# ZulutionAI/MoviiGen1.1

Measured on AMD Instinct MI355X. Metric: denoise-steps/sec, higher is better.
Workload: dtype bf16; 1 GPU; 14B T2V 1920x832x81f bf16 (the metric's configuration; BASELINE configs[2] shape); layers=40, parallelism=single, solver=unipc, weights=random N(0,0.02) bf16, seed 0

## Files before the change

### experiments/mfma_shape_probe.hip

```cpp
#include <hip/hip_runtime.h>
#include <stdio.h>
#include <stdlib.h>
#include <string.h>
#include <vector>

typedef __attribute__((ext_vector_type(8))) __bf16 bf16x8_t;
typedef __attribute__((ext_vector_type(16))) float f32x16_t;
typedef __attribute__((ext_vector_type(4))) float f32x4_t;
typedef __attribute__((ext_vector_type(4))) unsigned int u32x4_t;
#define CK(x) do { hipError_t e_ = (x); if (e_ != hipSuccess) { printf("HIP error %s at %d\n", hipGetErrorString(e_), __LINE__); exit(1); } } while (0)
#define SB() __builtin_amdgcn_sched_barrier(0)

template <int SHAPE, int FILL, int WAVES, int RDS = 1>
__global__ __launch_bounds__(WAVES * 64, 1) void mix(const u32x4_t* __restrict__ in, float* __restrict__ out, int iters,
                                                     unsigned long long* __restrict__ cyc) {
    __shared__ __attribute__((aligned(16))) char smem[96 * 1024];
    const int tid = threadIdx.x, lane = tid & 63;
    for (int i = tid; i < 4096; i += WAVES * 64) ((u32x4_t*)smem)[i] = in[i];
    __syncthreads();
    bf16x8_t a[4], b[4];
#pragma unroll
    for (int i = 0; i < 4; ++i) {
        a[i] = __builtin_bit_cast(bf16x8_t, in[(tid * 4 + i) & 4095]);
        b[i] = __builtin_bit_cast(bf16x8_t, in[(tid * 4 + i + 1777) & 4095]);
    }
    f32x16_t A32[4];
    f32x4_t A16[16];
#pragma unroll
    for (int i = 0; i < 4; ++i)
#pragma unroll
        for (int e = 0; e < 16; ++e) A32[i][e] = 0.f;
#pragma unroll
    for (int i = 0; i < 16; ++i) A16[i] = (f32x4_t){0.f, 0.f, 0.f, 0.f};
    float x[4] = {0.001f * lane, -0.002f * lane, 0.5f, -0.25f}, y[4] = {0, 0, 0, 0}, s0 = 0.f, s1 = 0.f;
    unsigned pk = 0;
    const char* lp = smem + lane * 16;
    auto fill_a = [&](int k) __attribute__((always_inline)) {
        asm volatile("v_exp_f32 %0, %1" : "=v"(y[k & 3]) : "v"(x[k & 3]));
        asm volatile("v_add_f32 %0, %0, %1" : "+v"(s0) : "v"(y[(k + 2) & 3]));
    };
    auto fill_b = [&](int k) __attribute__((always_inline)) {
        asm volatile("v_exp_f32 %0, %1" : "=v"(y[(k + 1) & 3]) : "v"(x[(k + 1) & 3]));
        asm volatile("v_add_f32 %0, %0, %1" : "+v"(s1) : "v"(y[(k + 3) & 3]));
        asm volatile("v_cvt_pk_bf16_f32 %0, %1, %2" : "=v"(pk) : "v"(y[k & 3]), "v"(y[(k + 2) & 3]));
    };
    const unsigned long long t0 = __builtin_amdgcn_s_memtime();
    for (int it = 0; it < iters; ++it) {
#pragma unroll
        for (int j = 0; j < 8; ++j) {
            if (SHAPE == 0) {
                A32[(2 * j) & 3] = __builtin_amdgcn_mfma_f32_32x32x16_bf16(a[j & 3], b[j & 3], A32[(2 * j) & 3], 0, 0, 0);
                SB();
#pragma unroll
                for (int f = 0; f < FILL; ++f) fill_a(j + f);
                SB();
                A32[(2 * j + 1) & 3] = __builtin_amdgcn_mfma_f32_32x32x16_bf16(a[j & 3], b[(j + 1) & 3], A32[(2 * j + 1) & 3], 0, 0, 0);
                SB();
#pragma unroll
                for (int f = 0; f < FILL; ++f) fill_b(j + f);
            } else {
                A16[(4 * j) & 15] = __builtin_amdgcn_mfma_f32_16x16x32_bf16(a[j & 3], b[j & 3], A16[(4 * j) & 15], 0, 0, 0);
                SB();
#pragma unroll
                for (int f = 0; f < FILL; ++f) asm volatile("v_exp_f32 %0, %1" : "=v"(y[(j + f) & 3]) : "v"(x[(j + f) & 3]));
                SB();
                A16[(4 * j + 1) & 15] = __builtin_amdgcn_mfma_f32_16x16x32_bf16(a[j & 3], b[(j + 1) & 3], A16[(4 * j + 1) & 15], 0, 0, 0);
                SB();
#pragma unroll
                for (int f = 0; f < FILL; ++f) {
                    asm volatile("v_add_f32 %0, %0, %1" : "+v"(s0) : "v"(y[(j + f + 2) & 3]));
                    asm volatile("v_add_f32 %0, %0, %1" : "+v"(s1) : "v"(y[(j + f + 3) & 3]));
                }
                SB();
                A16[(4 * j + 2) & 15] = __builtin_amdgcn_mfma_f32_16x16x32_bf16(a[j & 3], b[(j + 2) & 3], A16[(4 * j + 2) & 15], 0, 0, 0);
                SB();
#pragma unroll
                for (int f = 0; f < FILL; ++f) asm volatile("v_exp_f32 %0, %1" : "=v"(y[(j + f + 1) & 3]) : "v"(x[(j + f + 1) & 3]));
                SB();
                A16[(4 * j + 3) & 15] = __builtin_amdgcn_mfma_f32_16x16x32_bf16(a[j & 3], b[(j + 3) & 3], A16[(4 * j + 3) & 15], 0, 0, 0);
                SB();
#pragma unroll
                for (int f = 0; f < FILL; ++f)
                    asm volatile("v_cvt_pk_bf16_f32 %0, %1, %2" : "=v"(pk) : "v"(y[(j + f) & 3]), "v"(y[(j + f + 2) & 3]));
            }
            if (FILL >= 0) a[(j + 2) & 3] = *(const bf16x8_t*)(lp + ((j * 1024 + it * 8192) & 0xfc00));
            if (RDS >= 2) b[(j + 2) & 3] = *(const bf16x8_t*)(lp + ((j * 1024 + it * 8192 + 32768) & 0xfc00));
            SB();
        }
    }
    const unsigned long long t1 = __builtin_amdgcn_s_memtime();
    float r = s0 + s1 + __uint_as_float(pk);
#pragma unroll
    for (int i = 0; i < 4; ++i)
#pragma unroll
        for (int e = 0; e < 16; ++e) r += A32[i][e];
#pragma unroll
    for (int i = 0; i < 16; ++i) r += A16[i][0] + A16[i][1] + A16[i][2] + A16[i][3];
    out[blockIdx.x * WAVES * 64 + tid] = r;
    if (tid == 0) cyc[blockIdx.x] = t1 - t0;
}

template <int SHAPE, int FILL, int WAVES, int RDS = 1>
static void run(const u32x4_t* in, float* out, unsigned long long* cyc, int rounds) {
    const int iters = 20000, grid = 1024;
    for (int r = 0; r < rounds; ++r) {
        hipEvent_t e0, e1;
        CK(hipEventCreate(&e0)); CK(hipEventCreate(&e1));
        hipLaunchKernelGGL((mix<SHAPE, FILL, WAVES, RDS>), dim3(grid), dim3(WAVES * 64), 0, 0, in, out, 2000, cyc);
        CK(hipDeviceSynchronize());
        CK(hipEventRecord(e0));
        hipLaunchKernelGGL((mix<SHAPE, FILL, WAVES, RDS>), dim3(grid), dim3(WAVES * 64), 0, 0, in, out, iters, cyc);
        CK(hipEventRecord(e1));
        CK(hipEventSynchronize(e1));
        float ms;
        CK(hipEventElapsedTime(&ms, e0, e1));
        std::vector<unsigned long long> h(grid);
        CK(hipMemcpy(h.data(), cyc, grid * 8, hipMemcpyDeviceToHost));
        double cs = 0;
        for (auto v : h) cs += (double)v;
        cs /= grid;
        const double flops = (double)grid * WAVES * iters * 8 * 65536.0;
        printf("%s  waves/CU %d  fill x%d (VALU per 32x32x16-equivalent: %.1f) + %.1f ds_read: %8.1f TF/s  %6.1f cyc per 32768 FLOP  (clock ~%.2f GHz)\n",
               SHAPE ? "16x16x32" : "32x32x16", WAVES, FILL, FILL * 2.5, 0.5 * RDS, flops / (ms * 1e-3) / 1e12, cs / (iters * 16.0),
               cs * (grid / 256.0) / (ms * 1e-3) / 1e9 / 1.0);
        fflush(stdout);
    }
}

int main() {
    u32x4_t* in; float* out; unsigned long long* cyc;
    CK(hipMalloc(&in, 65536)); CK(hipMalloc(&out, 1024 * 512 * 4)); CK(hipMalloc(&cyc, 1024 * 8));
    std::vector<unsigned short> h(32768);
    srand(1);
    for (auto& v : h) {
        float f = ((rand() % 2001) - 1000) / 1000.0f;
        unsigned u; memcpy(&u, &f, 4);
        v = (unsigned short)(u >> 16);
    }
    CK(hipMemcpy(in, h.data(), 65536, hipMemcpyHostToDevice));
    for (int round = 0; round < 2; ++round) {
        run<0, 0, 4>(in, out, cyc, 1);
        run<1, 0, 4>(in, out, cyc, 1);
        run<0, 1, 4>(in, out, cyc, 1);
        run<1, 1, 4>(in, out, cyc, 1);
        run<0, 2, 4>(in, out, cyc, 1);
        run<1, 2, 4>(in, out, cyc, 1);
        run<0, 1, 8>(in, out, cyc, 1);
        run<1, 1, 8>(in, out, cyc, 1);
        run<1, 1, 8, 2>(in, out, cyc, 1);
        run<1, 1, 4, 2>(in, out, cyc, 1);
    }
    return 0;
}
```

### include/moviigen_hip.h

```cpp
#ifndef MOVIIGEN_HIP_H
#define MOVIIGEN_HIP_H

#include <stdint.h>

#ifdef __cplusplus
extern "C" {
#endif

#define MG_OK 0
#define MG_ERR_ARG (-1)
#define MG_ERR_SHAPE (-2)
#define MG_ERR_LAUNCH (-3)
#define MG_ERR_UNAVAILABLE (-4)
#define MG_ERR_COMM (-5)

const char* mg_version(void);
int mg_abi_version(void);


int mg_ln_modulate(const float* x, int64_t ldx, int64_t rows, int dim, const float* scale,
                   const float* shift, int add_one, float eps, int round_norm_bf16, void* out,
                   int out_f32, int64_t ldo, void* stream);

int64_t mg_step_resid_partials_bytes(void);
int mg_step_resid_capture_f32(float* r, const float* x, const float* xin, int64_t n, double* stats, double* partials,
                              void* stream);
int mg_resid_ln_modulate_f32(const float* x, int64_t ldx, const float* r, int64_t ldr, int64_t rows, int dim,
                             const float* scale, const float* shift, float eps, float* out, int64_t ldo, void* stream);

int mg_rmsnorm_rope_bf16(const uint16_t* x, int64_t ldx, uint16_t* out, int64_t ldo,
                         int64_t rows, int dim, const float* weight, float eps, int head_dim,
                         const float* rope_cs, int F, int H, int W, int64_t pos0, float out_scale, void* stream);

int mg_pack_kv_bf16(const uint16_t* k, int64_t ldk, const uint16_t* v, int64_t ldv, int64_t L,
                    int heads, int head_dim, uint16_t* kp, uint16_t* vp, void* stream);


enum {
    MG_EPI_BIAS_BF16 = 0,
    MG_EPI_BIAS_GELU_BF16 = 1,
    MG_EPI_GATE_RESID_F32 = 2,
    MG_EPI_BIAS_F32 = 3
};

int mg_gemm_bf16(const uint16_t* A, int64_t lda, const uint16_t* W, int64_t ldw,
                 const float* bias, int64_t M, int N, int K, int epilogue, void* out,
                 int64_t ldo, const float* gate, void* stream);

int mg_quant_mxfp8_rows(const uint16_t* x, int64_t ldx, int64_t rows, int K, uint8_t* q, int64_t ldq,
                        uint8_t* scales, int64_t lds, void* stream);

int mg_gemm_mxfp8(const uint8_t* Aq, int64_t lda, const uint8_t* As, int64_t ldas, const uint8_t* Wq, int64_t ldw,
                  const uint8_t* Ws, int64_t ldws, const float* bias, int64_t M, int N, int K, int epilogue,
                  void* out, int64_t ldo, const float* gate, void* stream);

int mg_ln_modulate_mxfp8(const float* x, int64_t ldx, int64_t rows, int dim, const float* scale, const float* shift,
                         int add_one, float eps, int round_norm_bf16, uint16_t* out, int64_t ldo, uint8_t* q,
                         int64_t ldq, uint8_t* scales, int64_t lds, void* stream);

int mg_gemm_mxfp8_gelu_q(const uint8_t* Aq, int64_t lda, const uint8_t* As, int64_t ldas, const uint8_t* Wq, int64_t ldw,
                         const uint8_t* Ws, int64_t ldws, const float* bias, int64_t M, int N, int K, uint8_t* oq,
                         int64_t ldoq, uint8_t* oscales, int64_t ldos, void* stream);

int64_t mg_attn_workspace_bytes(void);
int mg_attn_fwd_bf16_hd128(const uint16_t* q, int64_t ldq, const uint16_t* kp, const uint16_t* vp,
                           uint16_t* o, int64_t ldo, int64_t Lq, int64_t Lk, int heads, float scale,
                           void* workspace, void* stream);

int mg_attn_fwd_bf16_hd128_lse(const uint16_t* q, int64_t ldq, const uint16_t* kp, const uint16_t* vp,
                               uint16_t* o, int64_t ldo, float* lse, int64_t Lq, int64_t Lk, int heads,
                               float scale, void* workspace, void* stream);

int mg_attn_fwd_bf16_hd128_prescaled(const uint16_t* q, int64_t ldq, const uint16_t* kp, const uint16_t* vp,
                                     uint16_t* o, int64_t ldo, float* lse, int64_t Lq, int64_t Lk, int heads,
                                     int reserve_cus, void* workspace, void* stream);

int mg_gate_residual_f32(float* x, int64_t ldx, const uint16_t* y, int64_t ldy, const float* gate, int64_t rows,
                         int dim, void* stream);


int mg_sp_pack_qkv_bf16(const uint16_t* q, int64_t ldq, const uint16_t* k, int64_t ldk, const uint16_t* v,
                        int64_t ldv, int64_t Lloc, int P, int cols_per_dest, int col0, int w, uint16_t* send,
                        void* stream);

int mg_sp_unpack_o_bf16(const uint16_t* recv, int64_t Lloc, int P, int cols_per_src, int col0, int w, uint16_t* o,
                        int64_t ldo, void* stream);

int mg_sp_copy_blocks_bf16(const uint16_t* src, int64_t s_blk, int64_t s_row, uint16_t* dst, int64_t d_blk,
                           int64_t d_row, int blocks, int64_t rows, int width, void* stream);


int mg_comm_unique_id(void* id128);
int mg_comm_create(const void* id128, int nranks, int rank, void** comm);
int mg_comm_destroy(void* comm);

int mg_sp_all_to_all(void* comm, const void* send, void* recv, int64_t bytes_per_peer, void* stream);

int mg_sp_all_to_all_4d_bf16(void* comm, const uint16_t* x, int64_t ldx, int64_t rows, int heads, int head_dim,
                             int seq_to_head, uint16_t* out, int64_t ldo, uint16_t* workspace, void* stream);

int mg_sp_all_gather(void* comm, const void* send, void* recv, int64_t bytes, void* stream);
int mg_shard_all_gather(void* comm, const void* shard, void* full, int64_t shard_bytes, void* stream);

int mg_attn_merge_f32(float* acc, int64_t lda, float* lse_acc, const uint16_t* part, int64_t ldp,
                      const float* lse_part, uint16_t* out, int64_t ldo, int64_t Lq, int heads, int first,
                      void* stream);

int mg_attn_fwd_bf16_generic(const uint16_t* q, int64_t ldq, const uint16_t* k, int64_t ldk,
                             const uint16_t* v, int64_t ldv, uint16_t* o, int64_t ldo, int64_t Lq,
                             int64_t Lk, int heads, int head_dim, float scale, void* stream);


int mg_sinusoid_embed(const void* t, int t_dtype, int n, int dim, float* out, void* stream);

int mg_gemv_f32(const float* W, const float* bias, const float* x, float* y, int N, int K,
                int silu_in, void* stream);

int mg_add_rows_f32(const float* a, const float* b, float* out, int rows, int dim, int period,
                    void* stream);

int mg_head_gemm_f32(const float* x, int64_t ldx, const float* W, const float* bias, float* out,
                     int64_t M, int N, int K, void* stream);

int mg_patchify_bf16(const float* lat, int C, int F, int H, int W, int ph, int pw,
                     uint16_t* out, int64_t ldo, void* stream);

int mg_unpatchify_f32(const float* tok, int64_t ldt, int C, int F, int Hg, int Wg, int ph, int pw,
                      float* lat, void* stream);

int mg_lincomb4_f32(float* out, int64_t n, const float* x0, float c0, const float* x1, float c1,
                    const float* x2, float c2, const float* x3, float c3, void* stream);

int mg_cfg_combine_f32(float* out, const float* uncond, const float* cond, float guide_scale,
                       int64_t n, void* stream);


int mg_embed_rows_bf16(const uint16_t* table, int64_t vocab, int dim, const int64_t* ids, int n,
                       uint16_t* out, void* stream);

int mg_ew_bf16(const uint16_t* a, const uint16_t* b, uint16_t* out, int64_t n, int mode, void* stream);

int mg_t5_attn_bf16(const uint16_t* q, const uint16_t* k, const uint16_t* v, int64_t ld,
                    const uint16_t* rel_emb, const int* rel_bucket, uint16_t* o, int64_t ldo,
                    int64_t Lq, int64_t Lk, int heads, int head_dim, void* stream);


int mg_vae_conv_f32(const float* x, const float* cache, int tc, int T, int H, int W, int Cin,
                    const float* w, const float* bias, int Cout, int kt, int kh, int kw, int up2,
                    const float* residual, float* out, int mode, void* stream);

int mg_vae_upconv_fold_weights_f32(const float* w, int Cout, int Cin, float* wp, void* stream);
int mg_vae_upconv_phases_f32(const float* x, int T, int H, int W, int Cin, const float* wp, const float* bias, int Cout,
                             float* out, int mode, void* stream);

int mg_vae_conv_cols_f32(const float* x, const float* cache, int tc, int T, int H, int W, int Cin,
                         const float* w, const float* bias, int Cout, int kt, int kh, int kw,
                         const float* residual, float* out, int col0, int cols, int mode, void* stream);
int mg_vae_upconv_phases_cols_f32(const float* x, int T, int H, int W, int Cin, const float* wp, const float* bias, int Cout,
                                  float* out, int col0, int cols, int mode, void* stream);

#define MG_VAE_EXACT 0
#define MG_VAE_BF16X3 1
#define MG_VAE_TILE_128 (1 << 8)
#define MG_VAE_TILE_256 (2 << 8)

int mg_vae_rmsnorm_silu_f32(const float* x, const float* gamma, float* out, int64_t rows, int C,
                            int do_silu, void* stream);

int64_t mg_vae_attn_workspace_floats(int64_t L, int C);
int mg_vae_attn_f32(const float* qkv, float* out, int frames, int64_t L, int C, float* workspace,
                    void* stream);
int mg_vae_attn_rows_f32(const float* q, int64_t ldq, const float* k, const float* v, int64_t ldkv, float* out, int frames,
                         int64_t Lq, int64_t Lk, int C, float* workspace, void* stream);

int mg_vae_latent_in_f32(const float* z, const float* mean, const float* inv_std, int C, int T,
                         int H, int W, float* out, void* stream);
int mg_vae_video_out_f32(const float* x, int C, int T, int H, int W, float* out, int t_off,
                         int T_total, void* stream);

int mg_video_to_u8(const float* video, int T, int H, int W, float lo, float hi, uint8_t* frames,
                   void* stream);

int mg_image_to_u8(const float* image, int H, int W, float lo, float hi, uint8_t* pixels, void* stream);

int mg_video_from_u8(const uint8_t* frames, int T, int H0, int W0, int H, int W, float* video, void* stream);

int mg_vae_time_interleave_f32(const float* x, int T, int64_t HW, int C, float* out, void* stream);


int mg_vae_conv_strided_f32(const float* x, const float* cache, int tc, int T, int H, int W, int Cin, const float* w, const float* bias,
                            int Cout, int kt, int kh, int kw, int st, int sh, int sw, int pt0, int ph0, int ph1, int pw0, int pw1,
                            float* out, int mode, void* stream);

int mg_vae_conv_in3_f32(const float* xs, const float* cache, int tc, int T, int H, int W, const float* w, const float* bias, int Cout,
                        float* out, int mode, void* stream);

int mg_vae_video_in_f32(const float* video, int T, int H, int W, int t0, int n, float* out, void* stream);
int mg_vae_latent_out_f32(const float* x, int ldx, const float* mean, const float* inv_std, int C, int T, int H, int W, float* out,
                          void* stream);


int mg_lora_merge(void* w, int w_f32, int64_t ldw, int N, int K, const float* up, int64_t ldu, const float* down, int64_t ldd, int R,
                  void* stream);

#ifdef MG_AB_BUILD
int mg_gemm_set_variant(int variant);

int mg_attn_set_variant(int variant);

void mg_attn_w64_profile(unsigned long long* dev_buf);
void mg_attn_w64_debug(int flags);
void mg_attn_w64_flag_counter(unsigned* dev_counter);
void mg_gemm_debug_profile(unsigned long long* dev_buf);
void mg_gemm5_debug_profile(unsigned long long* dev_buf);
#endif

#ifdef __cplusplus
}
#endif
#endif
```

### moviigen1.1_amd/csrc/attn_hd128_m16.hip

```cpp
#include <type_traits>
#include "common.h"
#include "../../include/moviigen_hip.h"

#define M16_THREADS 256
#define M16_QB 256
#define M16_TILE 16384
#define M16_K(slot) ((slot) * M16_TILE)
#define M16_V(slot) (3 * M16_TILE + (slot) * M16_TILE)

MG_DEV bf16x8_t m16_bf(u32x4_t v) { return __builtin_bit_cast(bf16x8_t, v); }
struct M16State {
    f32x4_t ot[8][4];
    f32x4_t st[2][2][4];
    bf16x8_t pf[2][4];
    f32x4_t mq[4];
    float m_run[4], l_run[4];
    float psa[4], psb[4];
    int bad;
};

template <int OFF>
MG_DEV void m16_rd(bf16x8_t& dst, unsigned addr) {
    asm volatile("ds_read_b128 %0, %1 offset:%2" : "=v"(dst) : "v"(addr), "i"(OFF));
}
template <int N>
MG_DEV void m16_wait() {
    asm volatile("s_waitcnt lgkmcnt(%0)" ::"i"(N) : "memory");
}
MG_DEV void m16_mfma_s0(f32x4_t& acc, const bf16x8_t& a, const bf16x8_t& b, const f32x4_t& c) {
    asm volatile("v_mfma_f32_16x16x32_bf16 %0, %1, %2, %3" : "=&v"(acc) : "v"(a), "a"(b), "v"(c));
}
MG_DEV void m16_mfma_s(f32x4_t& acc, const bf16x8_t& a, const bf16x8_t& b) {
    asm volatile("v_mfma_f32_16x16x32_bf16 %0, %1, %2, %0" : "+v"(acc) : "v"(a), "a"(b));
}
MG_DEV void m16_mfma_s_after_valu(f32x4_t& acc, const bf16x8_t& a, const bf16x8_t& b) {
    asm volatile("s_nop 7\n\ts_nop 7\n\tv_mfma_f32_16x16x32_bf16 %0, %1, %2, %0" : "+v"(acc) : "v"(a), "a"(b));
}
constexpr int m16_koff(int i) { return (i >> 2) * 256 + (i & 3) * 4096; }
constexpr int m16_voff(int i) { return i * 256; }

template <int KB>
MG_DEV void m16_softmax_exact(M16State& s, float c) {
#pragma unroll
    for (int n = 0; n < 4; ++n) {
        float tmax = s.st[KB][0][n][0];
#pragma unroll
        for (int r = 1; r < 4; ++r) tmax = fmaxf(tmax, s.st[KB][0][n][r]);
#pragma unroll
        for (int r = 0; r < 4; ++r) tmax = fmaxf(tmax, s.st[KB][1][n][r]);
        tmax = fmaxf(tmax, __shfl_xor(tmax, 16, 64));
        tmax = fmaxf(tmax, __shfl_xor(tmax, 32, 64));
        const float m_new = fmaxf(s.m_run[n], tmax);
        float psum = 0.f;
        float p[8];
#pragma unroll
        for (int r = 0; r < 8; ++r) {
            p[r] = __builtin_amdgcn_exp2f((s.st[KB][r >> 2][n][r & 3] - m_new) * c);
            psum += p[r];
        }
        u32x4_t w;
#pragma unroll
        for (int e = 0; e < 4; ++e) w[e] = pack_bf2(p[2 * e], p[2 * e + 1]);
        s.pf[KB][n] = m16_bf(w);
        const float alpha = __builtin_amdgcn_exp2f((s.m_run[n] - m_new) * c);
        s.l_run[n] = s.l_run[n] * alpha + psum;
#pragma unroll
        for (int d = 0; d < 8; ++d)
#pragma unroll
            for (int e = 0; e < 4; ++e) s.ot[d][n][e] *= alpha;
        s.m_run[n] = m_new;
    }
}

template <int KB>
MG_DEV void m16_softmax_zero(M16State& s, float c) {
#pragma unroll
    for (int n = 0; n < 4; ++n) {
        float psum = 0.f;
        float p[8];
#pragma unroll
        for (int r = 0; r < 8; ++r) {
            p[r] = __builtin_amdgcn_exp2f(s.st[KB][r >> 2][n][r & 3] * c);
            psum += p[r];
        }
        u32x4_t w;
#pragma unroll
        for (int e = 0; e < 4; ++e) w[e] = pack_bf2(p[2 * e], p[2 * e + 1]);
        s.pf[KB][n] = m16_bf(w);
        s.l_run[n] += psum;
    }
}

template <int KB>
MG_DEV void m16_mask_init(M16State& s, int lim, int G, const f32x4_t (&base)[4]) {
#pragma unroll
    for (int blk = 0; blk < 2; ++blk)
#pragma unroll
        for (int n = 0; n < 4; ++n)
#pragma unroll
            for (int r = 0; r < 4; ++r) {
                const int key = KB * 32 + G * 8 + blk * 4 + r;
                s.st[KB][blk][n][r] = key >= lim ? -1e30f : base[n][0];
            }
}

template <int KB, int SMODE, bool PV, bool SM, bool SCALED, int ORD, int LKO = 0, int LVO = 0, int NKO = 0, int NVO = 0, typename Dma>
MG_DEV void m16_step(M16State& s, const bf16x8_t (&qf)[4][4], bf16x8_t (&kf)[4], bf16x8_t (&vf)[4], unsigned lds_k,
                     unsigned lds_v, unsigned nk, unsigned nv, float c, Dma dma) {
    constexpr int SB = 1 - KB;
    u32x4_t w[4];
    float pa[2] = {0.f, 0.f}, pb[2] = {0.f, 0.f};
    auto exp_a = [&](int i, int half) __attribute__((always_inline)) {
        if (SM) {
            const int pp = 2 * i + half, n = pp >> 2, wd = pp & 3;
            const float x = s.st[SB][wd >> 1][n][(wd & 1) * 2];
            pa[half] = __builtin_amdgcn_exp2f(SCALED ? x * c : x);
            asm volatile("" : "+v"(pa[half]));
        }
    };
    auto exp_b = [&](int i, int half) __attribute__((always_inline)) {
        if (SM) {
            const int pp = 2 * i + half, n = pp >> 2, wd = pp & 3;
            const float x = s.st[SB][wd >> 1][n][(wd & 1) * 2 + 1];
            pb[half] = __builtin_amdgcn_exp2f(SCALED ? x * c : x);
            asm volatile("" : "+v"(pb[half]));
        }
    };
    auto add_a = [&](int i, int half) __attribute__((always_inline)) {
        if (SM) {
            const int n = (2 * i + half) >> 2;
            s.psa[n] += pa[half];
            asm volatile("" : "+v"(s.psa[n]));
        }
    };
    auto add_b = [&](int i, int half) __attribute__((always_inline)) {
        if (SM) {
            const int n = (2 * i + half) >> 2;
            s.psb[n] += pb[half];
            asm volatile("" : "+v"(s.psb[n]));
        }
    };
    auto cvt = [&](int i, int half) __attribute__((always_inline)) {
        if (SM) {
            const int pp = 2 * i + half, n = pp >> 2, wd = pp & 3;
            unsigned pk = pack_bf2(pa[half], pb[half]);
            asm volatile("" : "+v"(pk));
            w[n][wd] = pk;
        }
    };
    auto S = [&](int i, int n) __attribute__((always_inline)) {
        const int blk = i >> 2, c = i & 3, r = i & 3;
        if (SMODE == 1 && c == 0) m16_mfma_s0(s.st[KB][blk][n], kf[r], qf[n][c], s.mq[n]);
        else if (SMODE == 2 && c == 0) m16_mfma_s_after_valu(s.st[KB][blk][n], kf[r], qf[n][c]);
        else if (SMODE != 0) m16_mfma_s(s.st[KB][blk][n], kf[r], qf[n][c]);
    };
    auto P = [&](int i, int n) __attribute__((always_inline)) {
        if (PV) s.ot[i][n] = __builtin_amdgcn_mfma_f32_16x16x32_bf16(vf[i & 3], s.pf[KB][n], s.ot[i][n], 0, 0, 0);
    };
    auto rdK = [&](int i) __attribute__((always_inline)) {
        const int r2 = (i + 2) & 3;
        if (SMODE == 0) asm volatile("" ::"v"(kf[r2]));
        if (i < 6) {
            switch (i) {
                case 0: m16_rd<m16_koff(2) + LKO>(kf[r2], lds_k); break;
                case 1: m16_rd<m16_koff(3) + LKO>(kf[r2], lds_k); break;
                case 2: m16_rd<m16_koff(4) + LKO>(kf[r2], lds_k); break;
                case 3: m16_rd<m16_koff(5) + LKO>(kf[r2], lds_k); break;
                case 4: m16_rd<m16_koff(6) + LKO>(kf[r2], lds_k); break;
                default: m16_rd<m16_koff(7) + LKO>(kf[r2], lds_k); break;
            }
        } else if (i == 6) m16_rd<m16_koff(0) + NKO>(kf[r2], nk);
        else m16_rd<m16_koff(1) + NKO>(kf[r2], nk);
    };
    auto rdV = [&](int i) __attribute__((always_inline)) {
        const int r2 = (i + 2) & 3;
        if (i < 6) {
            switch (i) {
                case 0: m16_rd<m16_voff(2) + LVO>(vf[r2], lds_v); break;
                case 1: m16_rd<m16_voff(3) + LVO>(vf[r2], lds_v); break;
                case 2: m16_rd<m16_voff(4) + LVO>(vf[r2], lds_v); break;
                case 3: m16_rd<m16_voff(5) + LVO>(vf[r2], lds_v); break;
                case 4: m16_rd<m16_voff(6) + LVO>(vf[r2], lds_v); break;
                default: m16_rd<m16_voff(7) + LVO>(vf[r2], lds_v); break;
            }
        } else if (i == 6) m16_rd<m16_voff(0) + NVO>(vf[r2], nv);
        else m16_rd<m16_voff(1) + NVO>(vf[r2], nv);
    };
#define M16_SB() __builtin_amdgcn_sched_barrier(0)
#pragma unroll
    for (int i = 0; i < 8; ++i) {
        m16_wait<2>();
        M16_SB();
        if constexpr (ORD == 0) {
            S(i, 0); M16_SB();
            exp_a(i, 0); exp_b(i, 0); M16_SB();
            P(i, 0); M16_SB();
            add_a(i, 0); add_b(i, 0); cvt(i, 0); M16_SB();
            S(i, 1); M16_SB();
            rdK(i); M16_SB();
            P(i, 1); M16_SB();
            rdV(i); M16_SB();
            S(i, 2); M16_SB();
            exp_a(i, 1); exp_b(i, 1); M16_SB();
            P(i, 2); M16_SB();
            add_a(i, 1); add_b(i, 1); cvt(i, 1); M16_SB();
            S(i, 3); M16_SB();
            dma(i); M16_SB();
            P(i, 3); M16_SB();
        } else if constexpr (ORD == 1) {
            S(i, 0); M16_SB();
            exp_a(i, 0); M16_SB();
            P(i, 0); M16_SB();
            exp_b(i, 0); M16_SB();
            S(i, 1); M16_SB();
            add_a(i, 0); add_b(i, 0); cvt(i, 0); M16_SB();
            P(i, 1); M16_SB();
            rdK(i); M16_SB(); rdV(i); M16_SB();
            S(i, 2); M16_SB();
            exp_a(i, 1); M16_SB();
            P(i, 2); M16_SB();
            exp_b(i, 1); M16_SB();
            S(i, 3); M16_SB();
            add_a(i, 1); add_b(i, 1); cvt(i, 1); M16_SB();
            P(i, 3); M16_SB();
            dma(i); M16_SB();
        } else if constexpr (ORD == 2) {
            S(i, 0); M16_SB();
            exp_a(i, 0); M16_SB(); rdK(i); M16_SB();
            P(i, 0); M16_SB();
            exp_b(i, 0); M16_SB(); rdV(i); M16_SB();
            S(i, 1); M16_SB();
            add_a(i, 0); add_b(i, 0); cvt(i, 0); M16_SB();
            P(i, 1); M16_SB();
            S(i, 2); M16_SB();
            exp_a(i, 1); M16_SB();
            P(i, 2); M16_SB();
            exp_b(i, 1); M16_SB();
            S(i, 3); M16_SB();
            add_a(i, 1); add_b(i, 1); cvt(i, 1); M16_SB();
            P(i, 3); M16_SB();
            dma(i); M16_SB();
        } else if constexpr (ORD == 4) {
            S(i, 0); M16_SB();
            exp_a(i, 0); M16_SB();
            P(i, 0); M16_SB();
            exp_b(i, 0); M16_SB();
            S(i, 1); M16_SB();
            add_a(i, 0); add_b(i, 0); M16_SB();
            P(i, 1); M16_SB();
            cvt(i, 0); M16_SB(); rdK(i); M16_SB(); rdV(i); M16_SB();
            S(i, 2); M16_SB();
            exp_a(i, 1); M16_SB();
            P(i, 2); M16_SB();
            exp_b(i, 1); M16_SB();
            S(i, 3); M16_SB();
            add_a(i, 1); add_b(i, 1); M16_SB();
            P(i, 3); M16_SB();
            cvt(i, 1); M16_SB(); dma(i); M16_SB();
        } else if constexpr (ORD == 5) {
            S(i, 0); M16_SB();
            exp_a(i, 0); M16_SB();
            P(i, 0); M16_SB();
            exp_b(i, 0); M16_SB();
            S(i, 1); M16_SB();
            add_a(i, 0); add_b(i, 0); cvt(i, 0); M16_SB();
            P(i, 1); M16_SB();
            rdK(i); M16_SB();
            S(i, 2); M16_SB();
            exp_a(i, 1); M16_SB();
            P(i, 2); M16_SB();
            exp_b(i, 1); M16_SB();
            S(i, 3); M16_SB();
            add_a(i, 1); add_b(i, 1); cvt(i, 1); M16_SB();
            P(i, 3); M16_SB();
            rdV(i); M16_SB(); dma(i); M16_SB();
        } else if constexpr (ORD == 8) {
            S(i, 0); M16_SB();
            exp_a(i, 0); M16_SB();
            S(i, 1); M16_SB();
            exp_b(i, 0); M16_SB();
            P(i, 0); M16_SB();
            add_a(i, 0); add_b(i, 0); cvt(i, 0); M16_SB();
            P(i, 1); M16_SB();
            rdK(i); M16_SB(); rdV(i); M16_SB();
            S(i, 2); M16_SB();
            exp_a(i, 1); M16_SB();
            S(i, 3); M16_SB();
            exp_b(i, 1); M16_SB();
            P(i, 2); M16_SB();
            add_a(i, 1); add_b(i, 1); cvt(i, 1); M16_SB();
            P(i, 3); M16_SB();
            dma(i); M16_SB();
        } else if constexpr (ORD == 9) {
            S(i, 0); M16_SB();
            exp_a(i, 0); M16_SB();
            S(i, 1); M16_SB();
            exp_b(i, 0); M16_SB();
            S(i, 2); M16_SB();
            add_a(i, 0); add_b(i, 0); cvt(i, 0); M16_SB();
            S(i, 3); M16_SB();
            rdK(i); M16_SB(); rdV(i); M16_SB();
            P(i, 0); M16_SB();
            exp_a(i, 1); M16_SB();
            P(i, 1); M16_SB();
            exp_b(i, 1); M16_SB();
            P(i, 2); M16_SB();
            add_a(i, 1); add_b(i, 1); cvt(i, 1); M16_SB();
            P(i, 3); M16_SB();
            dma(i); M16_SB();
        } else {
            S(i, 0); M16_SB();
            exp_a(i, 0); M16_SB();
            P(i, 0); M16_SB();
            exp_b(i, 0); M16_SB();
            S(i, 1); M16_SB();
            exp_a(i, 1); M16_SB();
            P(i, 1); M16_SB();
            exp_b(i, 1); M16_SB();
            S(i, 2); M16_SB();
            add_a(i, 0); add_b(i, 0); cvt(i, 0); M16_SB();
            P(i, 2); M16_SB();
            add_a(i, 1); add_b(i, 1); cvt(i, 1); M16_SB();
            S(i, 3); M16_SB();
            rdK(i); M16_SB(); rdV(i); M16_SB();
            P(i, 3); M16_SB();
            dma(i); M16_SB();
        }
    }
#undef M16_SB
    if (SM) {
#pragma unroll
        for (int n = 0; n < 4; ++n) {
            s.pf[SB][n] = m16_bf(w[n]);
        }
    }
}

MG_DEV int m16_lane() {
    int l;
    asm volatile("v_mbcnt_lo_u32_b32 %0, -1, 0\n\tv_mbcnt_hi_u32_b32 %0, -1, %0" : "=v"(l));
    return l;
}

struct M16NoDma {
    __device__ __forceinline__ void operator()(int) const {}
};

template <bool PROF, bool SCALED, int ORD>
__global__ __launch_bounds__(M16_THREADS, 1) void attn_hd128_m16_kernel(
    const uint16_t* __restrict__ q, int64_t ldq, const uint16_t* __restrict__ kp, const uint16_t* __restrict__ vp,
    uint16_t* __restrict__ o, int64_t ldo, int64_t Lq, int64_t Lk, int heads, float c_log2, int nqb, int dbg,
    unsigned long long* __restrict__ prof, float* __restrict__ lse, unsigned* __restrict__ flagcnt, unsigned* __restrict__ tickets) {
    __shared__ __attribute__((aligned(16))) char smem[6 * M16_TILE];
    __shared__ int s_next_item;
    const int bid = blockIdx.x;
    const unsigned long long r_start = PROF ? __builtin_amdgcn_s_memrealtime() : 0;
    const int tid = threadIdx.x;
    const int wave = __builtin_amdgcn_readfirstlane(tid >> 6);
    const int total_items = nqb * heads;
    const int nwg = gridDim.x;
    const bool ticketed = tickets != nullptr && nwg != total_items;
    int item, item_end, item_step;
    if (nwg == total_items || ticketed) {
        item = bid, item_end = ticketed ? total_items : bid + 1, item_step = 1;
    } else {
        const int xcd = bid & 7, slot = bid >> 3;
        item = (int)((int64_t)xcd * total_items / 8) + slot;
        item_end = (int)((int64_t)(xcd + 1) * total_items / 8);
        item_step = nwg >> 3;
    }
    unsigned next_ticket = 0;
    unsigned long long ph[8] = {0, 0, 0, 0, 0, 0, 0, 0}, ph_t = 0;
    unsigned long long pf_fence = 0, pf_a = 0, pf_b = 0, pf_n = 0;
    while (item < item_end) {
    if (ticketed && tid == 0) next_ticket = atomicAdd(tickets, 1u);
    const int head = item / nqb;
    const int qb0 = item - head * nqb;
    const int lane = m16_lane();
    int qi = lane & 15, G = lane >> 4;
    __syncthreads();
    if (PROF) ph_t = __builtin_amdgcn_s_memtime();

    bf16x8_t qf[4][4];
    const int64_t qrow_base = (int64_t)qb0 * M16_QB + wave * 64 + qi;
#pragma unroll
    for (int n = 0; n < 4; ++n) {
        const int64_t qr = qrow_base + n * 16;
        const int64_t qrow = qr < Lq ? qr : Lq - 1;
        const uint16_t* qp = q + qrow * ldq + head * 128 + G * 8;
#pragma unroll
        for (int c = 0; c < 4; ++c) qf[n][c] = m16_bf(*(const u32x4_t*)(qp + c * 32));
    }
    const int T = (int)((Lk + 63) / 64);
    const int last_lim = (int)(Lk - (int64_t)(T - 1) * 64);
    const int nfull = last_lim == 64 ? T : T - 1;
    const unsigned lds0 = (unsigned)(uintptr_t)(mg_lptr_t)smem;
    const uint64_t kb64 = (uint64_t)(uintptr_t)(kp + ((int64_t)head * T) * 8192), vb64 = (uint64_t)(uintptr_t)(vp + ((int64_t)head * T) * 8192);
    const u32x4_t rs_k = {(unsigned)__builtin_amdgcn_readfirstlane((int)(unsigned)kb64), (unsigned)__builtin_amdgcn_readfirstlane((int)((unsigned)(kb64 >> 32) & 0xffffu)),
                          (unsigned)T * M16_TILE, 0x00020000u};
    const u32x4_t rs_v = {(unsigned)__builtin_amdgcn_readfirstlane((int)(unsigned)vb64), (unsigned)__builtin_amdgcn_readfirstlane((int)((unsigned)(vb64 >> 32) & 0xffffu)),
                          (unsigned)T * M16_TILE, 0x00020000u};
    const int dvo = wave * 4096 + lane * 16;
    const unsigned lds_w = (unsigned)__builtin_amdgcn_readfirstlane((int)(lds0 + wave * 4096));
    auto dma_tile4 = [&](const u32x4_t& rs, int t, unsigned lbase) __attribute__((always_inline)) {
        const int soff = __builtin_amdgcn_readfirstlane((t < T ? t : T - 1) * M16_TILE);
        asm volatile("s_mov_b32 m0, %2\n\ts_nop 4\n\t"
                     "buffer_load_dwordx4 %0, %1, %3 offen lds\n\t"
                     "buffer_load_dwordx4 %0, %1, %3 offen offset:1024 lds\n\t"
                     "buffer_load_dwordx4 %0, %1, %3 offen offset:2048 lds\n\t"
                     "buffer_load_dwordx4 %0, %1, %3 offen offset:3072 lds"
                     :: "v"(dvo), "s"(rs), "s"(lbase), "s"(soff) : "memory");
    };
    auto dma_k4 = [&](int t, int slot) __attribute__((always_inline)) { dma_tile4(rs_k, t, lds_w + M16_K(slot)); };
    auto dma_v4 = [&](int t, int slot) __attribute__((always_inline)) { dma_tile4(rs_v, t, lds_w + M16_V(slot)); };
    unsigned kbase = lds0 + G * 1024 + qi * 16;
    unsigned vbase = lds0 + 3 * M16_TILE + G * 2048 + qi * 16;
    auto k_addr = [&](int slot, int kb) __attribute__((always_inline)) { return kbase + slot * M16_TILE + kb * 512; };
    auto v_addr = [&](int slot, int kb) __attribute__((always_inline)) { return vbase + slot * M16_TILE + kb * 8192; };

    M16State s;
    bf16x8_t kf[4], vf[4];
    auto reset = [&]() __attribute__((always_inline)) {
#pragma unroll
        for (int d = 0; d < 8; ++d)
#pragma unroll
            for (int n = 0; n < 4; ++n) s.ot[d][n] = (f32x4_t){0.f, 0.f, 0.f, 0.f};
#pragma unroll
        for (int n = 0; n < 4; ++n) s.m_run[n] = -1e30f, s.l_run[n] = 0.f, s.psa[n] = 0.f, s.psb[n] = 0.f;
        s.bad = 0;
    };
    reset();
    auto q_pin = [&]() __attribute__((always_inline)) {
#pragma unroll
        for (int n = 0; n < 4; ++n)
#pragma unroll
            for (int c = 0; c < 4; ++c) asm volatile("" : "+a"(qf[n][c]));
    };
    auto fence = [&]() __attribute__((always_inline)) {
        asm volatile("s_waitcnt vmcnt(0)" ::: "memory");
        __syncthreads();
    };
    auto fence_hot = [&]() __attribute__((always_inline)) {
        asm volatile("s_waitcnt vmcnt(0)\n\ts_barrier" ::: "memory");
    };
    auto prefetch = [&](unsigned ak, unsigned av) __attribute__((always_inline)) {
        m16_rd<m16_koff(0)>(kf[0], ak);
        m16_rd<m16_voff(0)>(vf[0], av);
        m16_rd<m16_koff(1)>(kf[1], ak);
        m16_rd<m16_voff(1)>(vf[1], av);
    };
    const f32x4_t zero4[4] = {{0.f, 0.f, 0.f, 0.f}, {0.f, 0.f, 0.f, 0.f}, {0.f, 0.f, 0.f, 0.f}, {0.f, 0.f, 0.f, 0.f}};
    auto bare_S = [&](auto kbc, int slot, int lim) __attribute__((always_inline)) {
        constexpr int KB = decltype(kbc)::value;
        if (lim < 64) m16_mask_init<KB>(s, lim, G, zero4);
        else {
#pragma unroll
            for (int blk = 0; blk < 2; ++blk)
#pragma unroll
                for (int n = 0; n < 4; ++n) s.st[KB][blk][n] = (f32x4_t){0.f, 0.f, 0.f, 0.f};
        }
        const char* base = smem + M16_K(slot) + G * 1024 + qi * 16 + KB * 512;
#pragma unroll
        for (int i = 0; i < 8; ++i) {
            const bf16x8_t f = *(const bf16x8_t*)(base + m16_koff(i));
#pragma unroll
            for (int n = 0; n < 4; ++n)
                s.st[KB][i >> 2][n] = __builtin_amdgcn_mfma_f32_16x16x32_bf16(f, qf[n][i & 3], s.st[KB][i >> 2][n], 0, 0, 0);
        }
    };
    auto bare_PV = [&](auto kbc, int slot) __attribute__((always_inline)) {
        constexpr int KB = decltype(kbc)::value;
        const char* base = smem + M16_V(slot) + G * 2048 + qi * 16 + KB * 8192;
#pragma unroll
        for (int i = 0; i < 8; ++i) {
            const bf16x8_t f = *(const bf16x8_t*)(base + m16_voff(i));
#pragma unroll
            for (int n = 0; n < 4; ++n)
                s.ot[i][n] = __builtin_amdgcn_mfma_f32_16x16x32_bf16(f, s.pf[KB][n], s.ot[i][n], 0, 0, 0);
        }
    };
    using KB0 = std::integral_constant<int, 0>;
    using KB1 = std::integral_constant<int, 1>;

    bool exact_pass = nfull < 3;
    if (!exact_pass) {
    for (int attempt = 0;; ++attempt) {
        auto tile_max = [&](float (&mx)[4]) __attribute__((always_inline)) {
#pragma unroll
            for (int n = 0; n < 4; ++n) {
                float a = fmaxf(fmaxf(s.st[0][0][n][0], s.st[0][0][n][1]), fmaxf(s.st[0][0][n][2], s.st[0][0][n][3]));
                float b = fmaxf(fmaxf(s.st[0][1][n][0], s.st[0][1][n][1]), fmaxf(s.st[0][1][n][2], s.st[0][1][n][3]));
                float c2 = fmaxf(fmaxf(s.st[1][0][n][0], s.st[1][0][n][1]), fmaxf(s.st[1][0][n][2], s.st[1][0][n][3]));
                float d2 = fmaxf(fmaxf(s.st[1][1][n][0], s.st[1][1][n][1]), fmaxf(s.st[1][1][n][2], s.st[1][1][n][3]));
                mx[n] = fmaxf(mx[n], fmaxf(fmaxf(a, b), fmaxf(c2, d2)));
            }
        };
        auto set_reference = [&](const float (&mx)[4], float above) __attribute__((always_inline)) {
#pragma unroll
            for (int n = 0; n < 4; ++n) {
                float m = fmaxf(mx[n], __shfl_xor(mx[n], 16, 64));
                m = fmaxf(m, __shfl_xor(m, 32, 64)) + above;
                s.mq[n] = (f32x4_t){-m, -m, -m, -m};
            }
        };
        if (attempt) {
            float mx[4] = {-1e30f, -1e30f, -1e30f, -1e30f};
#pragma unroll
            for (int a = 0; a < 4; ++a) dma_k4(a, a);
            for (int t = 0; t < T; ++t) {
                asm volatile("s_waitcnt vmcnt(12)" ::: "memory");
                __syncthreads();
                dma_k4(t + 4, (t + 4) % 6);
                const int lim = t == T - 1 ? last_lim : 64;
                bare_S(KB0{}, t % 6, lim);
                bare_S(KB1{}, t % 6, lim);
                tile_max(mx);
            }
            asm volatile("s_waitcnt vmcnt(0)" ::: "memory");
            set_reference(mx, 0.f);
            __syncthreads();
            reset();
        }
        dma_k4(0, 0), dma_v4(0, 0), dma_k4(1, 1);
        fence();
        q_pin();
        if (PROF) { const unsigned long long tt = __builtin_amdgcn_s_memtime(); ph[0] += tt - ph_t; ph_t = tt; }
        dma_k4(2, 2), dma_v4(1, 1);
        bare_S(KB0{}, 0, 64);
        bare_S(KB1{}, 0, 64);
        if (attempt == 0) {
            float mx[4] = {-1e30f, -1e30f, -1e30f, -1e30f};
            tile_max(mx);
            set_reference(mx, c_log2 > 1e-20f ? 64.f / c_log2 : 0.f);
        }
#pragma unroll
        for (int kb = 0; kb < 2; ++kb)
#pragma unroll
            for (int blk = 0; blk < 2; ++blk)
#pragma unroll
                for (int n = 0; n < 4; ++n) s.st[kb][blk][n] += s.mq[n];
        m16_softmax_zero<0>(s, c_log2);
#pragma unroll
        for (int n = 0; n < 4; ++n) asm volatile("" : "+v"(s.l_run[n]));
        prefetch(k_addr(1, 0), v_addr(0, 0));
        m16_step<0, 1, true, true, SCALED, ORD>(s, qf, kf, vf, k_addr(1, 0), v_addr(0, 0), k_addr(1, 1), v_addr(0, 1), c_log2, M16NoDma());
        int t = 1;
        unsigned ka0 = k_addr(0, 0), ka1 = k_addr(1, 0), ka2 = k_addr(2, 0);
        unsigned va0 = v_addr(0, 0), va1 = v_addr(1, 0), va2 = v_addr(2, 0);
        unsigned lk0 = (unsigned)__builtin_amdgcn_readfirstlane((int)(lds0 + M16_K(0) + wave * 4096));
        unsigned lk1 = lk0 + M16_TILE, lk2 = lk0 + 2 * M16_TILE;
        int offk = (t + 2) * M16_TILE, offv = (t + 1) * M16_TILE;
        unsigned keep_m0, rot_tmp;
#define M16_BDMA0(VOFF, RS, SOFF, LBASE, IMM)                                                                                              \
    asm volatile("s_add_u32 m0, %2, %3\n\ts_nop 0\n\tbuffer_load_dwordx4 %0, %1, %4 offen lds"                                             \
                 :: "v"(VOFF), "s"(RS), "s"(LBASE), "n"(IMM), "s"(SOFF) : "memory", "scc")
#define M16_BDMAN(VOFF, RS, SOFF, IMM)                                                                                                     \
    asm volatile("buffer_load_dwordx4 %0, %1, %3 offen offset:%2 lds" :: "v"(VOFF), "s"(RS), "n"(IMM), "s"(SOFF) : "memory")
        asm volatile("s_mov_b32 %0, m0\n\ts_nop 4" : "=s"(keep_m0) :: "memory");
        if (PROF) { const unsigned long long tt = __builtin_amdgcn_s_memtime(); ph[1] += tt - ph_t; ph_t = tt; }
        __builtin_amdgcn_s_waitcnt(0x0F70);
        asm volatile("" : "+v"(ka0), "+v"(ka1), "+v"(ka2), "+v"(va0), "+v"(va1), "+v"(va2));
        if (PROF) { const unsigned long long tt = __builtin_amdgcn_s_memtime(); ph[2] += tt - ph_t; ph_t = tt; }
        for (; t + 1 < nfull; ++t) {
            const unsigned long long c0 = PROF ? __builtin_amdgcn_s_memtime() : 0;
            fence_hot();
            const unsigned long long c1 = PROF ? __builtin_amdgcn_s_memtime() : 0;
            m16_step<1, 1, true, true, SCALED, ORD, 512, 8192, 0, 0>(s, qf, kf, vf, ka1, va0, ka2, va1, c_log2,
                                       [&](int n) __attribute__((always_inline)) {
                                           switch (n) {
                                               case 0: M16_BDMA0(dvo, rs_k, offk, lk0, 0); break;
                                               case 1: M16_BDMAN(dvo, rs_k, offk, 1024); break;
                                               case 2: M16_BDMAN(dvo, rs_k, offk, 2048); break;
                                               case 3: M16_BDMAN(dvo, rs_k, offk, 3072); break;
                                               case 4: M16_BDMA0(dvo, rs_v, offv, lk2, 3 * M16_TILE); break;
                                               case 5: M16_BDMAN(dvo, rs_v, offv, 1024); break;
                                               case 6: M16_BDMAN(dvo, rs_v, offv, 2048); break;
                                               default: M16_BDMAN(dvo, rs_v, offv, 3072); break;
                                           }
                                       });
            const unsigned long long c2 = PROF ? __builtin_amdgcn_s_memtime() : 0;
            m16_step<0, 1, true, true, SCALED, ORD, 0, 0, 512, 8192>(s, qf, kf, vf, ka2, va1, ka2, va1, c_log2,
                                       [&](int n) __attribute__((always_inline)) {
                                           if (n == 0)
                                               asm volatile("s_add_u32 %0, %0, 0x4000\n\ts_add_u32 %1, %1, 0x4000" : "+s"(offk), "+s"(offv) : : "scc");
                                           else if (n == 1)
                                               asm volatile("s_mov_b32 %3, %0\n\ts_mov_b32 %0, %1\n\ts_mov_b32 %1, %2\n\ts_mov_b32 %2, %3"
                                                            : "+s"(lk0), "+s"(lk1), "+s"(lk2), "=&s"(rot_tmp));
                                           else if (n == 7) {
                                               asm volatile("v_swap_b32 %0, %1\n\tv_swap_b32 %1, %2" : "+v"(ka0), "+v"(ka1), "+v"(ka2));
                                               asm volatile("v_swap_b32 %0, %1\n\tv_swap_b32 %1, %2" : "+v"(va0), "+v"(va1), "+v"(va2));
                                           }
                                       });
            if (PROF) {
                const unsigned long long c3 = __builtin_amdgcn_s_memtime();
                pf_fence += c1 - c0, pf_a += c2 - c1, pf_b += c3 - c2, pf_n += 1;
            }
        }
#undef M16_BDMA0
#undef M16_BDMAN
        asm volatile("s_mov_b32 m0, %0" :: "s"(keep_m0) : "memory");
        if (PROF) { const unsigned long long tt = __builtin_amdgcn_s_memtime(); ph[3] += tt - ph_t; ph_t = tt; }
        static_assert(M16_TILE == 0x4000, "the literal above");
        const int s0 = (t - 1) % 3, s1 = t % 3, s2 = (t + 1) % 3;
        {
            const int l2 = m16_lane();
            qi = l2 & 15, G = l2 >> 4;
            kbase = lds0 + G * 1024 + qi * 16;
            vbase = lds0 + 3 * M16_TILE + G * 2048 + qi * 16;
        }
        fence();
        if (t + 1 < T) {
            dma_v4(t + 1, s2);
        }
        m16_step<1, 1, true, true, SCALED, ORD>(s, qf, kf, vf, k_addr(s1, 1), v_addr(s0, 1), k_addr(s2, 0), v_addr(s1, 0), c_log2, M16NoDma());
        if (t + 1 < T) {
            m16_mask_init<0>(s, last_lim, G, s.mq);
            m16_step<0, 2, true, true, SCALED, ORD>(s, qf, kf, vf, k_addr(s2, 0), v_addr(s1, 0), k_addr(s2, 1), v_addr(s1, 1), c_log2, M16NoDma());
            fence();
            m16_mask_init<1>(s, last_lim, G, s.mq);
            m16_step<1, 2, true, true, SCALED, ORD>(s, qf, kf, vf, k_addr(s2, 1), v_addr(s1, 1), k_addr(s2, 1), v_addr(s2, 0), c_log2, M16NoDma());
            m16_step<0, 0, true, true, SCALED, ORD>(s, qf, kf, vf, k_addr(s2, 1), v_addr(s2, 0), k_addr(s2, 1), v_addr(s2, 1), c_log2, M16NoDma());
            m16_step<1, 0, true, false, SCALED, ORD>(s, qf, kf, vf, k_addr(s2, 1), v_addr(s2, 1), k_addr(s2, 1), v_addr(s2, 1), c_log2, M16NoDma());
        } else {
            m16_step<0, 0, true, true, SCALED, ORD>(s, qf, kf, vf, k_addr(s1, 1), v_addr(s1, 0), k_addr(s1, 1), v_addr(s1, 1), c_log2, M16NoDma());
            m16_step<1, 0, true, false, SCALED, ORD>(s, qf, kf, vf, k_addr(s1, 1), v_addr(s1, 1), k_addr(s1, 1), v_addr(s1, 1), c_log2, M16NoDma());
        }
        m16_wait<0>();
        asm volatile("" ::"v"(kf[0]), "v"(kf[1]), "v"(kf[2]), "v"(kf[3]), "v"(vf[0]), "v"(vf[1]), "v"(vf[2]), "v"(vf[3]));
#pragma unroll
        for (int n = 0; n < 4; ++n) {
            s.l_run[n] += s.psa[n] + s.psb[n];
            s.psa[n] = s.psb[n] = 0.f;
            float lt = s.l_run[n] + __shfl_xor(s.l_run[n], 16, 64);
            lt += __shfl_xor(lt, 32, 64);
            s.bad |= !(lt >= 8.4703295e-22f && lt <= 1.2379400e27f);
            s.m_run[n] = -s.mq[n][0];
        }
        const bool flagged = __syncthreads_or(s.bad) != 0;
        if (PROF) { const unsigned long long tt = __builtin_amdgcn_s_memtime(); ph[4] += tt - ph_t; ph_t = tt; }
        if (!flagged || (dbg & 1)) break;
        if (flagcnt && tid == 0) atomicAdd(flagcnt + (attempt ? 1 : 0), 1u);
        if (attempt) {
            exact_pass = true;
            break;
        }
    }
    }
    if (exact_pass) {
        reset();
        for (int t = 0; t < T; ++t) {
            __syncthreads();
            dma_k4(t, 0), dma_v4(t, 0);
            fence();
            q_pin();
            const int lim = t == T - 1 ? last_lim : 64;
            bare_S(KB0{}, 0, lim);
            bare_S(KB1{}, 0, lim);
            m16_softmax_exact<0>(s, c_log2);
            bare_PV(KB0{}, 0);
            m16_softmax_exact<1>(s, c_log2);
            bare_PV(KB1{}, 0);
        }
    }

    {
        const int l3 = m16_lane();
        qi = l3 & 15, G = l3 >> 4;
    }
#pragma unroll
    for (int n = 0; n < 4; ++n) {
        float l_tot = s.l_run[n] + __shfl_xor(s.l_run[n], 16, 64);
        l_tot += __shfl_xor(l_tot, 32, 64);
        const float inv = 1.f / l_tot;
        const int64_t qr = (int64_t)qb0 * M16_QB + wave * 64 + n * 16 + qi;
        if (lse && G == 0 && qr < Lq) lse[(int64_t)head * Lq + qr] = (s.m_run[n] * c_log2 + __log2f(l_tot)) * 0.6931471805599453f;
        if (qr < Lq) {
            uint16_t* op = o + qr * ldo + head * 128 + G * 4;
#pragma unroll
            for (int d = 0; d < 8; ++d) {
                uint2 pk;
                pk.x = pack_bf2(s.ot[d][n][0] * inv, s.ot[d][n][1] * inv);
                pk.y = pack_bf2(s.ot[d][n][2] * inv, s.ot[d][n][3] * inv);
                *(uint2*)(op + d * 16) = pk;
            }
        }
    }
    if (PROF) { ph[7] += __builtin_amdgcn_s_memtime() - ph_t; asm volatile("s_waitcnt vmcnt(0)" ::: "memory"); const unsigned long long tt = __builtin_amdgcn_s_memtime(); ph[5] += tt - ph_t; ph[6] += 1; }
    if (ticketed) {
        if (tid == 0) s_next_item = nwg + (int)next_ticket;
        __syncthreads();
        item = __builtin_amdgcn_readfirstlane(s_next_item);
    } else
        item += item_step;
    }
    if (ticketed && tid == 0 && atomicAdd(tickets + 1, 1u) == (unsigned)nwg - 1) {
        __hip_atomic_store(tickets, 0u, __ATOMIC_RELAXED, __HIP_MEMORY_SCOPE_AGENT);
        __hip_atomic_store(tickets + 1, 0u, __ATOMIC_RELAXED, __HIP_MEMORY_SCOPE_AGENT);
    }
    if (PROF && prof && tid == 0) prof[16 + 2 * bid] = r_start, prof[16 + 2 * bid + 1] = __builtin_amdgcn_s_memrealtime();
    if (PROF && prof && (tid & 63) == 0) {
        atomicAdd(prof + wave * 4 + 0, pf_fence);
        atomicAdd(prof + wave * 4 + 1, pf_a);
        atomicAdd(prof + wave * 4 + 2, pf_b);
        atomicAdd(prof + wave * 4 + 3, pf_n);
    }
    if (PROF && prof && tid == 0) {
#pragma unroll
        for (int i = 0; i < 8; ++i) atomicAdd(prof + 1040 + i, ph[i]);
    }
}

static int g_m16_dbg = 0;
static unsigned long long* g_m16_prof = nullptr;
static unsigned* g_m16_flagcnt = nullptr;
void mg_attn_m16_hooks(int dbg, unsigned long long* prof, unsigned* flagcnt) { g_m16_dbg = dbg, g_m16_prof = prof, g_m16_flagcnt = flagcnt; }

int mg_attn_m16_launch(const uint16_t* q, int64_t ldq, const uint16_t* kp, const uint16_t* vp, uint16_t* o, int64_t ldo,
                       int64_t Lq, int64_t Lk, int heads, float c_log2, int prescaled, int nqb, float* lse, int reserve_cus,
                       unsigned* workspace, hipStream_t st) {
    const int n_cu = mg_persistent_cus(reserve_cus);
    if (n_cu < 0) return MG_ERR_LAUNCH;
    const int total = nqb * heads;
    const unsigned grid = total <= n_cu ? (unsigned)total : (unsigned)n_cu;
    unsigned* tickets = nullptr;
    if (workspace && (int64_t)total >= 32 * (int64_t)grid && !(g_m16_dbg & 16))
        tickets = workspace;
#define M16_ORD 9
#define M16_LAUNCH(PROF, SCALED, ORD)                                                                                             \
    hipLaunchKernelGGL((attn_hd128_m16_kernel<PROF, SCALED, ORD>), dim3(grid), dim3(M16_THREADS), 0, st, q, ldq, kp, vp, o, ldo, Lq, \
                       Lk, heads, prescaled ? 1.0f : c_log2, nqb, g_m16_dbg, PROF ? g_m16_prof : nullptr, lse, g_m16_flagcnt, tickets)
#ifdef MG_AB_BUILD
    const int ord = (g_m16_dbg >> 1) & 7;
    const int mo = (g_m16_dbg >> 5) & 3;
    if (mo && prescaled && !g_m16_prof) {
        if (mo == 1) M16_LAUNCH(false, false, 8);
        else if (mo == 2) M16_LAUNCH(false, false, 9);
        else M16_LAUNCH(false, false, 1);
        return mg_check_launch();
    }
    if (ord && prescaled && !g_m16_prof) {
        if (ord == 1) M16_LAUNCH(false, false, 1);
        else if (ord == 2) M16_LAUNCH(false, false, 2);
        else if (ord == 3) M16_LAUNCH(false, false, 3);
        else if (ord == 4) M16_LAUNCH(false, false, 4);
        else if (ord == 5) M16_LAUNCH(false, false, 5);
        else M16_LAUNCH(false, false, 0);
        return mg_check_launch();
    }
#endif
    if (g_m16_prof) {
        if (prescaled) M16_LAUNCH(true, false, M16_ORD);
        else M16_LAUNCH(true, true, M16_ORD);
    } else {
        if (prescaled) M16_LAUNCH(false, false, M16_ORD);
        else M16_LAUNCH(false, true, M16_ORD);
    }
#undef M16_LAUNCH
    return mg_check_launch();
}
```

### moviigen1.1_amd/wan/backend/lib.py

```python
import ctypes
import os

_HERE = os.path.dirname(os.path.abspath(__file__))
LIB_PATH = os.path.normpath(os.path.join(_HERE, '..', '..', 'lib', 'libmoviigen_hip.so'))
LIB_AB_PATH = os.path.normpath(os.path.join(_HERE, '..', '..', 'lib', 'libmoviigen_hip_ab.so'))

c_i64, c_int, c_f32, c_vp = ctypes.c_int64, ctypes.c_int, ctypes.c_float, ctypes.c_void_p

SIGNATURES = {
    'mg_version': [],
    'mg_abi_version': [],
    'mg_ln_modulate': [c_vp, c_i64, c_i64, c_int, c_vp, c_vp, c_int, c_f32, c_int, c_vp, c_int, c_i64, c_vp],
    'mg_step_resid_partials_bytes': [],
    'mg_step_resid_capture_f32': [c_vp, c_vp, c_vp, c_i64, c_vp, c_vp, c_vp],
    'mg_resid_ln_modulate_f32': [c_vp, c_i64, c_vp, c_i64, c_i64, c_int, c_vp, c_vp, c_f32, c_vp, c_i64, c_vp],
    'mg_rmsnorm_rope_bf16': [c_vp, c_i64, c_vp, c_i64, c_i64, c_int, c_vp, c_f32, c_int, c_vp, c_int, c_int,
                             c_int, c_i64, c_f32, c_vp],
    'mg_pack_kv_bf16': [c_vp, c_i64, c_vp, c_i64, c_i64, c_int, c_int, c_vp, c_vp, c_vp],
    'mg_gemm_bf16': [c_vp, c_i64, c_vp, c_i64, c_vp, c_i64, c_int, c_int, c_int, c_vp, c_i64, c_vp, c_vp],
    'mg_quant_mxfp8_rows': [c_vp, c_i64, c_i64, c_int, c_vp, c_i64, c_vp, c_i64, c_vp],
    'mg_gemm_mxfp8': [c_vp, c_i64, c_vp, c_i64, c_vp, c_i64, c_vp, c_i64, c_vp, c_i64, c_int, c_int, c_int, c_vp, c_i64,
                      c_vp, c_vp],
    'mg_ln_modulate_mxfp8': [c_vp, c_i64, c_i64, c_int, c_vp, c_vp, c_int, c_f32, c_int, c_vp, c_i64, c_vp, c_i64, c_vp, c_i64, c_vp],
    'mg_gemm_mxfp8_gelu_q': [c_vp, c_i64, c_vp, c_i64, c_vp, c_i64, c_vp, c_i64, c_vp, c_i64, c_int, c_int, c_vp, c_i64, c_vp, c_i64,
                             c_vp],
    'mg_attn_workspace_bytes': [],
    'mg_attn_fwd_bf16_hd128': [c_vp, c_i64, c_vp, c_vp, c_vp, c_i64, c_i64, c_i64, c_int, c_f32, c_vp, c_vp],
    'mg_attn_fwd_bf16_hd128_lse': [c_vp, c_i64, c_vp, c_vp, c_vp, c_i64, c_vp, c_i64, c_i64, c_int, c_f32, c_vp, c_vp],
    'mg_attn_fwd_bf16_hd128_prescaled': [c_vp, c_i64, c_vp, c_vp, c_vp, c_i64, c_vp, c_i64, c_i64, c_int, c_int, c_vp, c_vp],
    'mg_attn_merge_f32': [c_vp, c_i64, c_vp, c_vp, c_i64, c_vp, c_vp, c_i64, c_i64, c_int, c_int, c_vp],
    'mg_attn_fwd_bf16_generic': [c_vp, c_i64, c_vp, c_i64, c_vp, c_i64, c_vp, c_i64, c_i64, c_i64, c_int, c_int,
                                 c_f32, c_vp],
    'mg_sinusoid_embed': [c_vp, c_int, c_int, c_int, c_vp, c_vp],
    'mg_gemv_f32': [c_vp, c_vp, c_vp, c_vp, c_int, c_int, c_int, c_vp],
    'mg_add_rows_f32': [c_vp, c_vp, c_vp, c_int, c_int, c_int, c_vp],
    'mg_head_gemm_f32': [c_vp, c_i64, c_vp, c_vp, c_vp, c_i64, c_int, c_int, c_vp],
    'mg_patchify_bf16': [c_vp, c_int, c_int, c_int, c_int, c_int, c_int, c_vp, c_i64, c_vp],
    'mg_unpatchify_f32': [c_vp, c_i64, c_int, c_int, c_int, c_int, c_int, c_int, c_vp, c_vp],
    'mg_lincomb4_f32': [c_vp, c_i64, c_vp, c_f32, c_vp, c_f32, c_vp, c_f32, c_vp, c_f32, c_vp],
    'mg_cfg_combine_f32': [c_vp, c_vp, c_vp, c_f32, c_i64, c_vp],
    'mg_embed_rows_bf16': [c_vp, c_i64, c_int, c_vp, c_int, c_vp, c_vp],
    'mg_ew_bf16': [c_vp, c_vp, c_vp, c_i64, c_int, c_vp],
    'mg_t5_attn_bf16': [c_vp, c_vp, c_vp, c_i64, c_vp, c_vp, c_vp, c_i64, c_i64, c_i64, c_int, c_int, c_vp],
    'mg_vae_conv_f32': [c_vp, c_vp, c_int, c_int, c_int, c_int, c_int, c_vp, c_vp, c_int, c_int, c_int, c_int,
                        c_int, c_vp, c_vp, c_int, c_vp],
    'mg_vae_upconv_fold_weights_f32': [c_vp, c_int, c_int, c_vp, c_vp],
    'mg_vae_upconv_phases_f32': [c_vp, c_int, c_int, c_int, c_int, c_vp, c_vp, c_int, c_vp, c_int, c_vp],
    'mg_vae_conv_cols_f32': [c_vp, c_vp, c_int, c_int, c_int, c_int, c_int, c_vp, c_vp, c_int, c_int, c_int, c_int,
                             c_vp, c_vp, c_int, c_int, c_int, c_vp],
    'mg_vae_upconv_phases_cols_f32': [c_vp, c_int, c_int, c_int, c_int, c_vp, c_vp, c_int, c_vp, c_int, c_int, c_int, c_vp],
    'mg_vae_rmsnorm_silu_f32': [c_vp, c_vp, c_vp, c_i64, c_int, c_int, c_vp],
    'mg_vae_attn_workspace_floats': [c_i64, c_int],
    'mg_vae_attn_f32': [c_vp, c_vp, c_int, c_i64, c_int, c_vp, c_vp],
    'mg_vae_attn_rows_f32': [c_vp, c_i64, c_vp, c_vp, c_i64, c_vp, c_int, c_i64, c_i64, c_int, c_vp, c_vp],
    'mg_vae_latent_in_f32': [c_vp, c_vp, c_vp, c_int, c_int, c_int, c_int, c_vp, c_vp],
    'mg_vae_video_out_f32': [c_vp, c_int, c_int, c_int, c_int, c_vp, c_int, c_int, c_vp],
    'mg_vae_time_interleave_f32': [c_vp, c_int, c_i64, c_int, c_vp, c_vp],
    'mg_vae_conv_strided_f32': [c_vp, c_vp, c_int, c_int, c_int, c_int, c_int, c_vp, c_vp, c_int, c_int, c_int, c_int,
                                c_int, c_int, c_int, c_int, c_int, c_int, c_int, c_int, c_vp, c_int, c_vp],
    'mg_vae_conv_in3_f32': [c_vp, c_vp, c_int, c_int, c_int, c_int, c_vp, c_vp, c_int, c_vp, c_int, c_vp],
    'mg_vae_video_in_f32': [c_vp, c_int, c_int, c_int, c_int, c_int, c_vp, c_vp],
    'mg_vae_latent_out_f32': [c_vp, c_int, c_vp, c_vp, c_int, c_int, c_int, c_int, c_vp, c_vp],
    'mg_video_to_u8': [c_vp, c_int, c_int, c_int, c_f32, c_f32, c_vp, c_vp],
    'mg_video_from_u8': [c_vp, c_int, c_int, c_int, c_int, c_int, c_vp, c_vp],
    'mg_lora_merge': [c_vp, c_int, c_i64, c_int, c_int, c_vp, c_i64, c_vp, c_i64, c_int, c_vp],
    'mg_comm_unique_id': [c_vp],
    'mg_comm_create': [c_vp, c_int, c_int, c_vp],
    'mg_comm_destroy': [c_vp],
    'mg_sp_all_to_all': [c_vp, c_vp, c_vp, c_i64, c_vp],
    'mg_sp_all_to_all_4d_bf16': [c_vp, c_vp, c_i64, c_i64, c_int, c_int, c_int, c_vp, c_i64, c_vp, c_vp],
    'mg_sp_all_gather': [c_vp, c_vp, c_vp, c_i64, c_vp],
    'mg_shard_all_gather': [c_vp, c_vp, c_vp, c_i64, c_vp],
    'mg_gate_residual_f32': [c_vp, c_i64, c_vp, c_i64, c_vp, c_i64, c_int, c_vp],
    'mg_image_to_u8': [c_vp, c_int, c_int, c_f32, c_f32, c_vp, c_vp],
    'mg_sp_pack_qkv_bf16': [c_vp, c_i64, c_vp, c_i64, c_vp, c_i64, c_i64, c_int, c_int, c_int, c_int, c_vp, c_vp],
    'mg_sp_copy_blocks_bf16': [c_vp, c_i64, c_i64, c_vp, c_i64, c_i64, c_int, c_i64, c_int, c_vp],
    'mg_sp_unpack_o_bf16': [c_vp, c_i64, c_int, c_int, c_int, c_int, c_vp, c_i64, c_vp],
}
SIGNATURES_AB = {
    'mg_attn_set_variant': [c_int],
    'mg_gemm_set_variant': [c_int],
    'mg_attn_w64_profile': [c_vp],
    'mg_attn_w64_debug': [c_int],
    'mg_attn_w64_flag_counter': [c_vp],
    'mg_gemm_debug_profile': [c_vp],
    'mg_gemm5_debug_profile': [c_vp],
}
_RESTYPE = {'mg_version': ctypes.c_char_p, 'mg_vae_attn_workspace_floats': ctypes.c_int64, 'mg_attn_workspace_bytes': ctypes.c_int64,
            'mg_step_resid_partials_bytes': ctypes.c_int64, 'mg_attn_w64_profile': None,
            'mg_attn_w64_debug': None, 'mg_attn_w64_flag_counter': None, 'mg_gemm_debug_profile': None, 'mg_gemm5_debug_profile': None}
DEFAULT_GEMM_VARIANT = 0

ERRORS = {-1: 'MG_ERR_ARG (null pointer / bad enum)', -2: 'MG_ERR_SHAPE (unsupported shape or alignment)',
          -3: 'MG_ERR_LAUNCH (kernel launch failed)', -4: 'MG_ERR_UNAVAILABLE (librccl could not be bound)',
          -5: 'MG_ERR_COMM (an RCCL call failed)'}

_lib = None
_lib_ab = None
_use_ab = False
DEFAULT_ATTN_VARIANT = 0


class MoviigenHipError(RuntimeError):
    pass


def _open(path, sigs):
    if not os.path.exists(path):
        raise MoviigenHipError(
            f'{path} not found: build it with `python __graft_entry__.py build` '
            '(hipcc --offload-arch=gfx950); there is no CPU/torch fallback for the hot path')
    lib = ctypes.CDLL(path)
    for name, args in sigs.items():
        fn = getattr(lib, name)
        fn.argtypes = args
        fn.restype = _RESTYPE.get(name, ctypes.c_int)
    return lib


def load():
    global _lib
    if _use_ab:
        return load_ab()
    if _lib is None:
        _lib = _open(LIB_PATH, SIGNATURES)
    return _lib


def load_ab():
    global _lib_ab
    if _lib_ab is None:
        _lib_ab = _open(LIB_AB_PATH, {**SIGNATURES, **SIGNATURES_AB})
    return _lib_ab


class ab_library:

    def __enter__(self):
        global _use_ab
        self._prev, _use_ab = _use_ab, True
        return load_ab()

    def __exit__(self, *exc):
        global _use_ab
        if self._prev:
            return False
        h = load_ab()
        h.mg_attn_set_variant(DEFAULT_ATTN_VARIANT)
        h.mg_gemm_set_variant(DEFAULT_GEMM_VARIANT)
        h.mg_attn_w64_debug(0)
        h.mg_attn_w64_profile(None)
        h.mg_attn_w64_flag_counter(None)
        h.mg_gemm_debug_profile(None)
        h.mg_gemm5_debug_profile(None)
        _use_ab = self._prev
        return False


def call(name, *args):
    rc = getattr(load(), name)(*args)
    if rc != 0:
        raise MoviigenHipError(f'{name} failed: {ERRORS.get(rc, rc)}')
```

Before: 0.04704 steps/s.

## Add five-query-block variant to hd128 attention kernel for long sequences

Templates the m16 flash-attention kernel on the number of 16-row query blocks per wave and adds an NB=5 path (320 query rows per workgroup) with its own MFMA/softmax interleaving. This raises the amount of work done per K/V tile loaded into LDS, cutting LDS read traffic per FLOP. It is auto-selected when Lk is large and there are enough work items per CU. The cost is higher register/AGPR pressure, explicit nops for MFMA hazards and a more intricate schedule. A probe mode is added to the MFMA microbenchmark to measure LDS read-rate sensitivity.

```diff
diff --git a/experiments/mfma_shape_probe.hip b/experiments/mfma_shape_probe.hip
--- a/experiments/mfma_shape_probe.hip
+++ b/experiments/mfma_shape_probe.hip
@@ -11,12 +11,12 @@
 #define CK(x) do { hipError_t e_ = (x); if (e_ != hipSuccess) { printf("HIP error %s at %d\n", hipGetErrorString(e_), __LINE__); exit(1); } } while (0)
 #define SB() __builtin_amdgcn_sched_barrier(0)
 
-template <int SHAPE, int FILL, int WAVES, int RDS = 1>
+template <int SHAPE, int FILL, int WAVES, int RDS = 1, int NG = 8, int RN = NG>
 __global__ __launch_bounds__(WAVES * 64, 1) void mix(const u32x4_t* __restrict__ in, float* __restrict__ out, int iters,
                                                      unsigned long long* __restrict__ cyc) {
     __shared__ __attribute__((aligned(16))) char smem[96 * 1024];
     const int tid = threadIdx.x, lane = tid & 63;
-    for (int i = tid; i < 4096; i += WAVES * 64) ((u32x4_t*)smem)[i] = in[i];
+    for (int i = tid; i < 6144; i += WAVES * 64) ((u32x4_t*)smem)[i] = in[i & 4095];
     __syncthreads();
     bf16x8_t a[4], b[4];
 #pragma unroll
@@ -47,7 +47,7 @@
     const unsigned long long t0 = __builtin_amdgcn_s_memtime();
     for (int it = 0; it < iters; ++it) {
 #pragma unroll
-        for (int j = 0; j < 8; ++j) {
+        for (int j = 0; j < NG; ++j) {
             if (SHAPE == 0) {
                 A32[(2 * j) & 3] = __builtin_amdgcn_mfma_f32_32x32x16_bf16(a[j & 3], b[j & 3], A32[(2 * j) & 3], 0, 0, 0);
                 SB();
@@ -83,7 +83,8 @@
                 for (int f = 0; f < FILL; ++f)
                     asm volatile("v_cvt_pk_bf16_f32 %0, %1, %2" : "=v"(pk) : "v"(y[(j + f) & 3]), "v"(y[(j + f + 2) & 3]));
             }
-            if (FILL >= 0) a[(j + 2) & 3] = *(const bf16x8_t*)(lp + ((j * 1024 + it * 8192) & 0xfc00));
+            if (FILL >= 0 && (j + 1) * RN / NG > j * RN / NG) a[(j + 2) & 3] = *(const bf16x8_t*)(NG == 8 ? lp + ((j * 1024 + it * 8192) & 0xfc00)
+                                                                                                  : lp + ((it * 8192) & 0xe000) + j * 1024);
             if (RDS >= 2) b[(j + 2) & 3] = *(const bf16x8_t*)(lp + ((j * 1024 + it * 8192 + 32768) & 0xfc00));
             SB();
         }
@@ -100,16 +101,16 @@
     if (tid == 0) cyc[blockIdx.x] = t1 - t0;
 }
 
-template <int SHAPE, int FILL, int WAVES, int RDS = 1>
-static void run(const u32x4_t* in, float* out, unsigned long long* cyc, int rounds) {
-    const int iters = 20000, grid = 1024;
+template <int SHAPE, int FILL, int WAVES, int RDS = 1, int NG = 8, int RN = NG>
+static void run(const u32x4_t* in, float* out, unsigned long long* cyc, int rounds, int longer = 1) {
+    const int iters = 160000 / NG * longer, grid = 1024;
     for (int r = 0; r < rounds; ++r) {
         hipEvent_t e0, e1;
         CK(hipEventCreate(&e0)); CK(hipEventCreate(&e1));
-        hipLaunchKernelGGL((mix<SHAPE, FILL, WAVES, RDS>), dim3(grid), dim3(WAVES * 64), 0, 0, in, out, 2000, cyc);
+        hipLaunchKernelGGL((mix<SHAPE, FILL, WAVES, RDS, NG, RN>), dim3(grid), dim3(WAVES * 64), 0, 0, in, out, 2000, cyc);
         CK(hipDeviceSynchronize());
         CK(hipEventRecord(e0));
-        hipLaunchKernelGGL((mix<SHAPE, FILL, WAVES, RDS>), dim3(grid), dim3(WAVES * 64), 0, 0, in, out, iters, cyc);
+        hipLaunchKernelGGL((mix<SHAPE, FILL, WAVES, RDS, NG, RN>), dim3(grid), dim3(WAVES * 64), 0, 0, in, out, iters, cyc);
         CK(hipEventRecord(e1));
         CK(hipEventSynchronize(e1));
         float ms;
@@ -119,15 +120,15 @@
         double cs = 0;
         for (auto v : h) cs += (double)v;
         cs /= grid;
-        const double flops = (double)grid * WAVES * iters * 8 * 65536.0;
-        printf("%s  waves/CU %d  fill x%d (VALU per 32x32x16-equivalent: %.1f) + %.1f ds_read: %8.1f TF/s  %6.1f cyc per 32768 FLOP  (clock ~%.2f GHz)\n",
-               SHAPE ? "16x16x32" : "32x32x16", WAVES, FILL, FILL * 2.5, 0.5 * RDS, flops / (ms * 1e-3) / 1e12, cs / (iters * 16.0),
+        const double flops = (double)grid * WAVES * iters * NG * 65536.0;
+        printf("%s  waves/CU %d  fill x%d (VALU per 32x32x16-equivalent: %.1f) + %.2f ds_read: %8.1f TF/s  %6.1f cyc per 32768 FLOP  (clock ~%.2f GHz)\n",
+               SHAPE ? "16x16x32" : "32x32x16", WAVES, FILL, FILL * 2.5, 0.5 * RDS * RN / NG, flops / (ms * 1e-3) / 1e12, cs / (iters * 2.0 * NG),
                cs * (grid / 256.0) / (ms * 1e-3) / 1e9 / 1.0);
         fflush(stdout);
     }
 }
 
-int main() {
+int main(int argc, char** argv) {
     u32x4_t* in; float* out; unsigned long long* cyc;
     CK(hipMalloc(&in, 65536)); CK(hipMalloc(&out, 1024 * 512 * 4)); CK(hipMalloc(&cyc, 1024 * 8));
     std::vector<unsigned short> h(32768);
@@ -138,6 +139,15 @@
         v = (unsigned short)(u >> 16);
     }
     CK(hipMemcpy(in, h.data(), 65536, hipMemcpyHostToDevice));
+    if (argc > 1 && !strcmp(argv[1], "readrate")) {
+        const int rounds = argc > 2 ? atoi(argv[2]) : 5;
+        for (int round = 0; round < rounds; ++round) {
+            run<1, 1, 4, 1, 20, 20>(in, out, cyc, 1, 8);
+            run<1, 1, 4, 1, 20, 16>(in, out, cyc, 1, 8);
+            run<1, 1, 4, 1, 20, 10>(in, out, cyc, 1, 8);
+        }
+        return 0;
+    }
     for (int round = 0; round < 2; ++round) {
         run<0, 0, 4>(in, out, cyc, 1);
         run<1, 0, 4>(in, out, cyc, 1);
diff --git a/include/moviigen_hip.h b/include/moviigen_hip.h
--- a/include/moviigen_hip.h
+++ b/include/moviigen_hip.h
@@ -208,6 +208,8 @@
 
 int mg_attn_set_variant(int variant);
 
+int mg_attn_set_query_blocks(int nb);
+
 void mg_attn_w64_profile(unsigned long long* dev_buf);
 void mg_attn_w64_debug(int flags);
 void mg_attn_w64_flag_counter(unsigned* dev_counter);
diff --git a/moviigen1.1_amd/csrc/attn_hd128_m16.hip b/moviigen1.1_amd/csrc/attn_hd128_m16.hip
--- a/moviigen1.1_amd/csrc/attn_hd128_m16.hip
+++ b/moviigen1.1_amd/csrc/attn_hd128_m16.hip
@@ -3,21 +3,25 @@
 #include "../../include/moviigen_hip.h"
 
 #define M16_THREADS 256
-#define M16_QB 256
 #define M16_TILE 16384
 #define M16_K(slot) ((slot) * M16_TILE)
 #define M16_V(slot) (3 * M16_TILE + (slot) * M16_TILE)
 
 MG_DEV bf16x8_t m16_bf(u32x4_t v) { return __builtin_bit_cast(bf16x8_t, v); }
+template <int NB>
 struct M16State {
-    f32x4_t ot[8][4];
-    f32x4_t st[2][2][4];
-    bf16x8_t pf[2][4];
-    f32x4_t mq[4];
-    float m_run[4], l_run[4];
-    float psa[4], psb[4];
+    f32x4_t ot[8][NB];
+    f32x4_t st[2][2][NB];
+    bf16x8_t pf[2][NB];
+    f32x4_t mq[NB];
+    float m_run[NB], l_run[NB];
+    float psa[NB], psb[NB];
     int bad;
 };
+
+template <int NB> struct M16RowMax;
+template <> struct M16RowMax<4> { float v[4] = {-1e30f, -1e30f, -1e30f, -1e30f}; };
+template <> struct M16RowMax<5> { float v[5] = {-1e30f, -1e30f, -1e30f, -1e30f, -1e30f}; };
 
 template <int OFF>
 MG_DEV void m16_rd(bf16x8_t& dst, unsigned addr) {
@@ -39,10 +43,10 @@
 constexpr int m16_koff(int i) { return (i >> 2) * 256 + (i & 3) * 4096; }
 constexpr int m16_voff(int i) { return i * 256; }
 
-template <int KB>
-MG_DEV void m16_softmax_exact(M16State& s, float c) {
-#pragma unroll
-    for (int n = 0; n < 4; ++n) {
+template <int KB, int NB>
+MG_DEV void m16_softmax_exact(M16State<NB>& s, float c) {
+#pragma unroll
+    for (int n = 0; n < NB; ++n) {
         float tmax = s.st[KB][0][n][0];
 #pragma unroll
         for (int r = 1; r < 4; ++r) tmax = fmaxf(tmax, s.st[KB][0][n][r]);
@@ -72,10 +76,10 @@
     }
 }
 
-template <int KB>
-MG_DEV void m16_softmax_zero(M16State& s, float c) {
-#pragma unroll
-    for (int n = 0; n < 4; ++n) {
+template <int KB, int NB>
+MG_DEV void m16_softmax_zero(M16State<NB>& s, float c) {
+#pragma unroll
+    for (int n = 0; n < NB; ++n) {
         float psum = 0.f;
         float p[8];
 #pragma unroll
@@ -91,12 +95,12 @@
     }
 }
 
-template <int KB>
-MG_DEV void m16_mask_init(M16State& s, int lim, int G, const f32x4_t (&base)[4]) {
+template <int KB, int NB>
+MG_DEV void m16_mask_init(M16State<NB>& s, int lim, int G, const f32x4_t (&base)[NB]) {
 #pragma unroll
     for (int blk = 0; blk < 2; ++blk)
 #pragma unroll
-        for (int n = 0; n < 4; ++n)
+        for (int n = 0; n < NB; ++n)
 #pragma unroll
             for (int r = 0; r < 4; ++r) {
                 const int key = KB * 32 + G * 8 + blk * 4 + r;
@@ -104,15 +108,18 @@
             }
 }
 
-template <int KB, int SMODE, bool PV, bool SM, bool SCALED, int ORD, int LKO = 0, int LVO = 0, int NKO = 0, int NVO = 0, typename Dma>
-MG_DEV void m16_step(M16State& s, const bf16x8_t (&qf)[4][4], bf16x8_t (&kf)[4], bf16x8_t (&vf)[4], unsigned lds_k,
+template <int KB, int SMODE, bool PV, bool SM, bool SCALED, int ORD, int LKO = 0, int LVO = 0, int NKO = 0, int NVO = 0, int NB, typename Dma>
+MG_DEV void m16_step(M16State<NB>& s, const bf16x8_t (&qf)[NB][4], bf16x8_t (&kf)[4], bf16x8_t (&vf)[4], unsigned lds_k,
                      unsigned lds_v, unsigned nk, unsigned nv, float c, Dma dma) {
+    static_assert(NB == 4 || (NB == 5 && ORD == 9), "five query blocks: the shipped placement only");
     constexpr int SB = 1 - KB;
-    u32x4_t w[4];
-    float pa[2] = {0.f, 0.f}, pb[2] = {0.f, 0.f};
+    constexpr int NH = NB == 4 ? 2 : 3;
+    u32x4_t w[NB];
+    float pa[NH] = {}, pb[NH] = {};
+    auto pair0 = [](int i) __attribute__((always_inline)) { return NB == 4 ? 2 * i : (5 * i) >> 1; };
     auto exp_a = [&](int i, int half) __attribute__((always_inline)) {
         if (SM) {
-            const int pp = 2 * i + half, n = pp >> 2, wd = pp & 3;
+            const int pp = pair0(i) + half, n = pp >> 2, wd = pp & 3;
             const float x = s.st[SB][wd >> 1][n][(wd & 1) * 2];
             pa[half] = __builtin_amdgcn_exp2f(SCALED ? x * c : x);
             asm volatile("" : "+v"(pa[half]));
@@ -120,7 +127,7 @@
     };
     auto exp_b = [&](int i, int half) __attribute__((always_inline)) {
         if (SM) {
-            const int pp = 2 * i + half, n = pp >> 2, wd = pp & 3;
+            const int pp = pair0(i) + half, n = pp >> 2, wd = pp & 3;
             const float x = s.st[SB][wd >> 1][n][(wd & 1) * 2 + 1];
             pb[half] = __builtin_amdgcn_exp2f(SCALED ? x * c : x);
             asm volatile("" : "+v"(pb[half]));
@@ -128,21 +135,21 @@
     };
     auto add_a = [&](int i, int half) __attribute__((always_inline)) {
         if (SM) {
-            const int n = (2 * i + half) >> 2;
+            const int n = (pair0(i) + half) >> 2;
             s.psa[n] += pa[half];
             asm volatile("" : "+v"(s.psa[n]));
         }
     };
     auto add_b = [&](int i, int half) __attribute__((always_inline)) {
         if (SM) {
-            const int n = (2 * i + half) >> 2;
+            const int n = (pair0(i) + half) >> 2;
             s.psb[n] += pb[half];
             asm volatile("" : "+v"(s.psb[n]));
         }
     };
     auto cvt = [&](int i, int half) __attribute__((always_inline)) {
         if (SM) {
-            const int pp = 2 * i + half, n = pp >> 2, wd = pp & 3;
+            const int pp = pair0(i) + half, n = pp >> 2, wd = pp & 3;
             unsigned pk = pack_bf2(pa[half], pb[half]);
             asm volatile("" : "+v"(pk));
             w[n][wd] = pk;
@@ -291,6 +298,28 @@
             add_a(i, 1); add_b(i, 1); cvt(i, 1); M16_SB();
             P(i, 3); M16_SB();
             dma(i); M16_SB();
+        } else if constexpr (ORD == 9 && NB == 5) {
+            S(i, 0); M16_SB();
+            exp_a(i, 0); M16_SB();
+            S(i, 1); M16_SB();
+            exp_b(i, 0); M16_SB();
+            S(i, 2); M16_SB();
+            add_a(i, 0); add_b(i, 0); cvt(i, 0); M16_SB();
+            S(i, 3); M16_SB();
+            rdK(i); M16_SB(); rdV(i); M16_SB();
+            S(i, 4); M16_SB();
+            exp_a(i, 1); M16_SB();
+            P(i, 0); M16_SB();
+            exp_b(i, 1); M16_SB();
+            P(i, 1); M16_SB();
+            add_a(i, 1); add_b(i, 1); cvt(i, 1); M16_SB();
+            P(i, 2); M16_SB();
+            if (i & 1) { exp_a(i, 2); M16_SB(); }
+            P(i, 3); M16_SB();
+            if (i & 1) { exp_b(i, 2); M16_SB(); }
+            P(i, 4); M16_SB();
+            if (i & 1) { add_a(i, 2); add_b(i, 2); cvt(i, 2); M16_SB(); }
+            dma(i); M16_SB();
         } else if constexpr (ORD == 9) {
             S(i, 0); M16_SB();
             exp_a(i, 0); M16_SB();
@@ -330,7 +359,7 @@
 #undef M16_SB
     if (SM) {
 #pragma unroll
-        for (int n = 0; n < 4; ++n) {
+        for (int n = 0; n < NB; ++n) {
             s.pf[SB][n] = m16_bf(w[n]);
         }
     }
@@ -346,7 +375,7 @@
     __device__ __forceinline__ void operator()(int) const {}
 };
 
-template <bool PROF, bool SCALED, int ORD>
+template <int NB, bool PROF, bool SCALED, int ORD>
 __global__ __launch_bounds__(M16_THREADS, 1) void attn_hd128_m16_kernel(
     const uint16_t* __restrict__ q, int64_t ldq, const uint16_t* __restrict__ kp, const uint16_t* __restrict__ vp,
     uint16_t* __restrict__ o, int64_t ldo, int64_t Lq, int64_t Lk, int heads, float c_log2, int nqb, int dbg,
@@ -381,10 +410,10 @@
     __syncthreads();
     if (PROF) ph_t = __builtin_amdgcn_s_memtime();
 
-    bf16x8_t qf[4][4];
-    const int64_t qrow_base = (int64_t)qb0 * M16_QB + wave * 64 + qi;
-#pragma unroll
-    for (int n = 0; n < 4; ++n) {
+    bf16x8_t qf[NB][4];
+    const int64_t qrow_base = (int64_t)qb0 * (64 * NB) + wave * (16 * NB) + qi;
+#pragma unroll
+    for (int n = 0; n < NB; ++n) {
         const int64_t qr = qrow_base + n * 16;
         const int64_t qrow = qr < Lq ? qr : Lq - 1;
         const uint16_t* qp = q + qrow * ldq + head * 128 + G * 8;
@@ -418,21 +447,27 @@
     auto k_addr = [&](int slot, int kb) __attribute__((always_inline)) { return kbase + slot * M16_TILE + kb * 512; };
     auto v_addr = [&](int slot, int kb) __attribute__((always_inline)) { return vbase + slot * M16_TILE + kb * 8192; };
 
-    M16State s;
+    M16State<NB> s;
     bf16x8_t kf[4], vf[4];
+    auto zero_ot = [&]() __attribute__((always_inline)) {
+#pragma unroll
+        for (int d = 0; d < 8; ++d)
+#pragma unroll
+            for (int n = 0; n < NB; ++n) {
+                s.ot[d][n] = (f32x4_t){0.f, 0.f, 0.f, 0.f};
+                if constexpr (NB != 4) asm volatile("" : "+a"(s.ot[d][n]));
+            }
+    };
     auto reset = [&]() __attribute__((always_inline)) {
-#pragma unroll
-        for (int d = 0; d < 8; ++d)
-#pragma unroll
-            for (int n = 0; n < 4; ++n) s.ot[d][n] = (f32x4_t){0.f, 0.f, 0.f, 0.f};
-#pragma unroll
-        for (int n = 0; n < 4; ++n) s.m_run[n] = -1e30f, s.l_run[n] = 0.f, s.psa[n] = 0.f, s.psb[n] = 0.f;
+        if constexpr (NB == 4) zero_ot();
+#pragma unroll
+        for (int n = 0; n < NB; ++n) s.m_run[n] = -1e30f, s.l_run[n] = 0.f, s.psa[n] = 0.f, s.psb[n] = 0.f;
         s.bad = 0;
     };
     reset();
     auto q_pin = [&]() __attribute__((always_inline)) {
 #pragma unroll
-        for (int n = 0; n < 4; ++n)
+        for (int n = 0; n < NB; ++n)
 #pragma unroll
             for (int c = 0; c < 4; ++c) asm volatile("" : "+a"(qf[n][c]));
     };
@@ -449,7 +484,7 @@
         m16_rd<m16_koff(1)>(kf[1], ak);
         m16_rd<m16_voff(1)>(vf[1], av);
     };
-    const f32x4_t zero4[4] = {{0.f, 0.f, 0.f, 0.f}, {0.f, 0.f, 0.f, 0.f}, {0.f, 0.f, 0.f, 0.f}, {0.f, 0.f, 0.f, 0.f}};
+    const f32x4_t zero4[NB] = {};
     auto bare_S = [&](auto kbc, int slot, int lim) __attribute__((always_inline)) {
         constexpr int KB = decltype(kbc)::value;
         if (lim < 64) m16_mask_init<KB>(s, lim, G, zero4);
@@ -457,15 +492,24 @@
 #pragma unroll
             for (int blk = 0; blk < 2; ++blk)
 #pragma unroll
-                for (int n = 0; n < 4; ++n) s.st[KB][blk][n] = (f32x4_t){0.f, 0.f, 0.f, 0.f};
+                for (int n = 0; n < NB; ++n) s.st[KB][blk][n] = (f32x4_t){0.f, 0.f, 0.f, 0.f};
         }
         const char* base = smem + M16_K(slot) + G * 1024 + qi * 16 + KB * 512;
 #pragma unroll
         for (int i = 0; i < 8; ++i) {
             const bf16x8_t f = *(const bf16x8_t*)(base + m16_koff(i));
 #pragma unroll
-            for (int n = 0; n < 4; ++n)
-                s.st[KB][i >> 2][n] = __builtin_amdgcn_mfma_f32_16x16x32_bf16(f, qf[n][i & 3], s.st[KB][i >> 2][n], 0, 0, 0);
+            for (int n = 0; n < NB; ++n) {
+                if constexpr (NB == 4)
+                    s.st[KB][i >> 2][n] = __builtin_amdgcn_mfma_f32_16x16x32_bf16(f, qf[n][i & 3], s.st[KB][i >> 2][n], 0, 0, 0);
+                else if ((i & 3) == 0) m16_mfma_s_after_valu(s.st[KB][i >> 2][n], f, qf[n][i & 3]);
+                else m16_mfma_s(s.st[KB][i >> 2][n], f, qf[n][i & 3]);
+            }
+        }
+        if constexpr (NB != 4) {
+            asm volatile("s_nop 7\n\ts_nop 7\n\ts_nop 3"
+                         : "+v"(s.st[KB][0][0]), "+v"(s.st[KB][0][1]), "+v"(s.st[KB][0][2]), "+v"(s.st[KB][0][3]), "+v"(s.st[KB][0][NB - 1]),
+                           "+v"(s.st[KB][1][0]), "+v"(s.st[KB][1][1]), "+v"(s.st[KB][1][2]), "+v"(s.st[KB][1][3]), "+v"(s.st[KB][1][NB - 1]));
         }
     };
     auto bare_PV = [&](auto kbc, int slot) __attribute__((always_inline)) {
@@ -475,7 +519,7 @@
         for (int i = 0; i < 8; ++i) {
             const bf16x8_t f = *(const bf16x8_t*)(base + m16_voff(i));
 #pragma unroll
-            for (int n = 0; n < 4; ++n)
+            for (int n = 0; n < NB; ++n)
                 s.ot[i][n] = __builtin_amdgcn_mfma_f32_16x16x32_bf16(f, s.pf[KB][n], s.ot[i][n], 0, 0, 0);
         }
     };
@@ -485,9 +529,9 @@
     bool exact_pass = nfull < 3;
     if (!exact_pass) {
     for (int attempt = 0;; ++attempt) {
-        auto tile_max = [&](float (&mx)[4]) __attribute__((always_inline)) {
-#pragma unroll
-            for (int n = 0; n < 4; ++n) {
+        auto tile_max = [&](float (&mx)[NB]) __attribute__((always_inline)) {
+#pragma unroll
+            for (int n = 0; n < NB; ++n) {
                 float a = fmaxf(fmaxf(s.st[0][0][n][0], s.st[0][0][n][1]), fmaxf(s.st[0][0][n][2], s.st[0][0][n][3]));
                 float b = fmaxf(fmaxf(s.st[0][1][n][0], s.st[0][1][n][1]), fmaxf(s.st[0][1][n][2], s.st[0][1][n][3]));
                 float c2 = fmaxf(fmaxf(s.st[1][0][n][0], s.st[1][0][n][1]), fmaxf(s.st[1][0][n][2], s.st[1][0][n][3]));
@@ -495,16 +539,17 @@
                 mx[n] = fmaxf(mx[n], fmaxf(fmaxf(a, b), fmaxf(c2, d2)));
             }
         };
-        auto set_reference = [&](const float (&mx)[4], float above) __attribute__((always_inline)) {
-#pragma unroll
-            for (int n = 0; n < 4; ++n) {
+        auto set_reference = [&](const float (&mx)[NB], float above) __attribute__((always_inline)) {
+#pragma unroll
+            for (int n = 0; n < NB; ++n) {
                 float m = fmaxf(mx[n], __shfl_xor(mx[n], 16, 64));
                 m = fmaxf(m, __shfl_xor(m, 32, 64)) + above;
                 s.mq[n] = (f32x4_t){-m, -m, -m, -m};
             }
         };
         if (attempt) {
-            float mx[4] = {-1e30f, -1e30f, -1e30f, -1e30f};
+            M16RowMax<NB> mx0;
+            float (&mx)[NB] = mx0.v;
 #pragma unroll
             for (int a = 0; a < 4; ++a) dma_k4(a, a);
             for (int t = 0; t < T; ++t) {
@@ -529,7 +574,8 @@
         bare_S(KB0{}, 0, 64);
         bare_S(KB1{}, 0, 64);
         if (attempt == 0) {
-            float mx[4] = {-1e30f, -1e30f, -1e30f, -1e30f};
+            M16RowMax<NB> mx0;
+            float (&mx)[NB] = mx0.v;
             tile_max(mx);
             set_reference(mx, c_log2 > 1e-20f ? 64.f / c_log2 : 0.f);
         }
@@ -538,10 +584,11 @@
 #pragma unroll
             for (int blk = 0; blk < 2; ++blk)
 #pragma unroll
-                for (int n = 0; n < 4; ++n) s.st[kb][blk][n] += s.mq[n];
+                for (int n = 0; n < NB; ++n) s.st[kb][blk][n] += s.mq[n];
         m16_softmax_zero<0>(s, c_log2);
 #pragma unroll
-        for (int n = 0; n < 4; ++n) asm volatile("" : "+v"(s.l_run[n]));
+        for (int n = 0; n < NB; ++n) asm volatile("" : "+v"(s.l_run[n]));
+        if constexpr (NB != 4) zero_ot();
         prefetch(k_addr(1, 0), v_addr(0, 0));
         m16_step<0, 1, true, true, SCALED, ORD>(s, qf, kf, vf, k_addr(1, 0), v_addr(0, 0), k_addr(1, 1), v_addr(0, 1), c_log2, M16NoDma());
         int t = 1;
@@ -628,7 +675,7 @@
         m16_wait<0>();
         asm volatile("" ::"v"(kf[0]), "v"(kf[1]), "v"(kf[2]), "v"(kf[3]), "v"(vf[0]), "v"(vf[1]), "v"(vf[2]), "v"(vf[3]));
 #pragma unroll
-        for (int n = 0; n < 4; ++n) {
+        for (int n = 0; n < NB; ++n) {
             s.l_run[n] += s.psa[n] + s.psb[n];
             s.psa[n] = s.psb[n] = 0.f;
             float lt = s.l_run[n] + __shfl_xor(s.l_run[n], 16, 64);
@@ -648,6 +695,7 @@
     }
     if (exact_pass) {
         reset();
+        if constexpr (NB != 4) zero_ot();
         for (int t = 0; t < T; ++t) {
             __syncthreads();
             dma_k4(t, 0), dma_v4(t, 0);
@@ -668,11 +716,11 @@
         qi = l3 & 15, G = l3 >> 4;
     }
 #pragma unroll
-    for (int n = 0; n < 4; ++n) {
+    for (int n = 0; n < NB; ++n) {
         float l_tot = s.l_run[n] + __shfl_xor(s.l_run[n], 16, 64);
         l_tot += __shfl_xor(l_tot, 32, 64);
         const float inv = 1.f / l_tot;
-        const int64_t qr = (int64_t)qb0 * M16_QB + wave * 64 + n * 16 + qi;
+        const int64_t qr = (int64_t)qb0 * (64 * NB) + wave * (16 * NB) + n * 16 + qi;
         if (lse && G == 0 && qr < Lq) lse[(int64_t)head * Lq + qr] = (s.m_run[n] * c_log2 + __log2f(l_tot)) * 0.6931471805599453f;
         if (qr < Lq) {
             uint16_t* op = o + qr * ldo + head * 128 + G * 4;
@@ -715,20 +763,49 @@
 static unsigned* g_m16_flagcnt = nullptr;
 void mg_attn_m16_hooks(int dbg, unsigned long long* prof, unsigned* flagcnt) { g_m16_dbg = dbg, g_m16_prof = prof, g_m16_flagcnt = flagcnt; }
 
+#ifdef MG_AB_BUILD
+static int g_m16_nb = 0;
+extern "C" int mg_attn_set_query_blocks(int nb) {
+    if (nb != 0 && nb != 4 && nb != 5) return MG_ERR_ARG;
+    g_m16_nb = nb;
+    return MG_OK;
+}
+#else
+static constexpr int g_m16_nb = 0;
+#endif
+static int m16_auto_nb(int64_t Lq, int64_t Lk, int heads, int n_cu, const unsigned* workspace) {
+    if (!workspace || Lk < 1024 * 64) return 4;
+    const int64_t items = (Lq + 319) / 320 * heads;
+    return items >= 32 * (int64_t)n_cu ? 5 : 4;
+}
+
 int mg_attn_m16_launch(const uint16_t* q, int64_t ldq, const uint16_t* kp, const uint16_t* vp, uint16_t* o, int64_t ldo,
                        int64_t Lq, int64_t Lk, int heads, float c_log2, int prescaled, int nqb, float* lse, int reserve_cus,
                        unsigned* workspace, hipStream_t st) {
     const int n_cu = mg_persistent_cus(reserve_cus);
     if (n_cu < 0) return MG_ERR_LAUNCH;
+    const int nb = g_m16_nb ? g_m16_nb : m16_auto_nb(Lq, Lk, heads, n_cu, workspace);
+    if (nb != 4) nqb = (int)((Lq + 64 * nb - 1) / (64 * nb));
     const int total = nqb * heads;
     const unsigned grid = total <= n_cu ? (unsigned)total : (unsigned)n_cu;
     unsigned* tickets = nullptr;
     if (workspace && (int64_t)total >= 32 * (int64_t)grid && !(g_m16_dbg & 16))
         tickets = workspace;
 #define M16_ORD 9
-#define M16_LAUNCH(PROF, SCALED, ORD)                                                                                             \
-    hipLaunchKernelGGL((attn_hd128_m16_kernel<PROF, SCALED, ORD>), dim3(grid), dim3(M16_THREADS), 0, st, q, ldq, kp, vp, o, ldo, Lq, \
+#define M16_LAUNCH_NB(NB, PROF, SCALED, ORD)                                                                                      \
+    hipLaunchKernelGGL((attn_hd128_m16_kernel<NB, PROF, SCALED, ORD>), dim3(grid), dim3(M16_THREADS), 0, st, q, ldq, kp, vp, o, ldo, Lq, \
                        Lk, heads, prescaled ? 1.0f : c_log2, nqb, g_m16_dbg, PROF ? g_m16_prof : nullptr, lse, g_m16_flagcnt, tickets)
+#define M16_LAUNCH(PROF, SCALED, ORD) M16_LAUNCH_NB(4, PROF, SCALED, ORD)
+    if (nb == 5) {
+        if (g_m16_prof) {
+            if (prescaled) M16_LAUNCH_NB(5, true, false, M16_ORD);
+            else M16_LAUNCH_NB(5, true, true, M16_ORD);
+        } else {
+            if (prescaled) M16_LAUNCH_NB(5, false, false, M16_ORD);
+            else M16_LAUNCH_NB(5, false, true, M16_ORD);
+        }
+        return mg_check_launch();
+    }
 #ifdef MG_AB_BUILD
     const int ord = (g_m16_dbg >> 1) & 7;
     const int mo = (g_m16_dbg >> 5) & 3;
@@ -756,5 +833,6 @@
         else M16_LAUNCH(false, true, M16_ORD);
     }
 #undef M16_LAUNCH
+#undef M16_LAUNCH_NB
     return mg_check_launch();
 }
diff --git a/moviigen1.1_amd/wan/backend/lib.py b/moviigen1.1_amd/wan/backend/lib.py
--- a/moviigen1.1_amd/wan/backend/lib.py
+++ b/moviigen1.1_amd/wan/backend/lib.py
@@ -79,6 +79,7 @@
 }
 SIGNATURES_AB = {
     'mg_attn_set_variant': [c_int],
+    'mg_attn_set_query_blocks': [c_int],
     'mg_gemm_set_variant': [c_int],
     'mg_attn_w64_profile': [c_vp],
     'mg_attn_w64_debug': [c_int],
@@ -99,6 +100,7 @@
 _lib_ab = None
 _use_ab = False
 DEFAULT_ATTN_VARIANT = 0
+DEFAULT_ATTN_QUERY_BLOCKS = 0
 
 
 class MoviigenHipError(RuntimeError):
@@ -147,6 +149,7 @@
             return False
         h = load_ab()
         h.mg_attn_set_variant(DEFAULT_ATTN_VARIANT)
+        h.mg_attn_set_query_blocks(DEFAULT_ATTN_QUERY_BLOCKS)
         h.mg_gemm_set_variant(DEFAULT_GEMM_VARIANT)
         h.mg_attn_w64_debug(0)
         h.mg_attn_w64_profile(None)
```

Measured after the change: 0.04749 steps/s, median of 6. No clear change (+0.9%).
